# Guilucand/PanDelos

Measured on AMD Instinct MI355X. Metric: scored gene-pairs/sec (whole node), higher is better.
Workload: dtype u32 accumulate + f32 finalize

## Files before the change

pandelos_amd/csrc/pdl_api.hip:

```cpp
#include "pdl_common.h"

#include <algorithm>
#include <cstdlib>
#include <cstring>
#include <limits>

static thread_local std::string g_create_error = "";

enum class Lock { held, take };
template <class Body, class Undo>
static int guarded(pdl_ctx *c, Lock lock, Body &&body, Undo &&undo) {
    int code = PDL_ERR_DEVICE;
    std::string msg;
    try { return body(); }
    catch (const pdl_error &e) { code = e.code; msg = e.msg; }
    catch (const std::bad_alloc &) { msg = "host allocation failed"; }
    catch (const std::exception &e) { msg = e.what(); }
    undo();
    if (!c) g_create_error = msg;
    else if (lock == Lock::take) { std::lock_guard<std::mutex> lk(c->mu); c->err = msg; }
    else c->err = msg;
    return code;
}
template <class Body> static int guarded(pdl_ctx *c, Body &&body) { return guarded(c, Lock::held, body, [] {}); }
// ... 574 lines not shown
    memset(out, 0, sizeof(*out));
    std::lock_guard<std::mutex> lk(c->mu);
    return guarded(c, Lock::held, [&]() -> int {
        if ((n_edges && (!src || !dst)) || (n_sequences && !genome_of)) PDL_FAIL(PDL_ERR_ARGUMENT, "pdl_families_of_edges: NULL pointer");
        if (n_edges >= 0x7fffffffull || n_sequences >= 0x7fffffffu) PDL_FAIL(PDL_ERR_UNSUPPORTED, "pdl_families_of_edges: 2^31 genes or edges and more");
        PDL_HIP(hipSetDevice(c->device));
        pdl_ctx::FamBufs &b = c->fb;
        uint32_t g_max = 0;
        for (uint32_t i = 0; i < n_sequences; i++) g_max = std::max(g_max, genome_of[i]);
        if (n_edges) {
            b.up_src.alloc(n_edges * 4); b.up_dst.alloc(n_edges * 4);
            PDL_HIP(hipMemcpyAsync(b.up_src.p, src, n_edges * 4, hipMemcpyHostToDevice, c->stream));
            PDL_HIP(hipMemcpyAsync(b.up_dst.p, dst, n_edges * 4, hipMemcpyHostToDevice, c->stream));
        }
        if (n_sequences) {
            b.up_gen.alloc((size_t) n_sequences * 4);
            PDL_HIP(hipMemcpyAsync(b.up_gen.p, genome_of, (size_t) n_sequences * 4, hipMemcpyHostToDevice, c->stream));
        }
        const int32_t *s2[2] = {b.up_src.as<int32_t>(), nullptr}, *d2[2] = {b.up_dst.as<int32_t>(), nullptr};
        const uint64_t n2[2] = {n_edges, 0};
        pdl_fam_result r;
        pdl_run_families(c, s2, d2, n2, false, true, true, b.up_gen.as<uint32_t>(), n_sequences, bit_length64(g_max), r);
        fill_families(r, out);
        return PDL_OK;
    }, [&] { pdl_free_families(out); });
}

void pdl_free_placement(pdl_placement *p) {
    if (!p) return;
    free(p->src); free(p->dst); free(p->score); free(p->family_of); free(p->is_node); free(p->group_label); free(p->group_query_off);
    free(p->group_query); free(p->group_base_off); free(p->group_base); free(p->group_collides);
    memset(p, 0, sizeof(*p));
}

static void fill_placement(const pdl_place_result &r, bool with_edges, pdl_placement *out) {
    out->sequences = r.sequences; out->n_query = r.n_query; out->genomes = r.genomes;
    out->edges = (uint32_t) r.src.size(); out->edges_phase1 = r.edges_phase1; out->groups = r.groups;
    out->novel = r.novel; out->joined = r.joined; out->bridging = r.bridging; out->colliding = r.colliding; out->unplaced = r.unplaced;
    out->device_ms = r.device_ms;
    if (with_edges) { out->src = dup_vec(r.src); out->dst = dup_vec(r.dst); out->score = dup_vec(r.score); }
    out->family_of = dup_vec(r.family_of); out->is_node = dup_vec(r.is_node); out->group_label = dup_vec(r.group_label);
    out->group_query_off = dup_vec(r.group_query_off); out->group_query = dup_vec(r.group_query);
    out->group_base_off = dup_vec(r.group_base_off); out->group_base = dup_vec(r.group_base); out->group_collides = dup_vec(r.group_collides);
}

int pdl_place_query(pdl_ctx *c, const uint8_t *residues, const uint64_t *offsets, uint32_t n_query, pdl_placement *out, pdl_query_info *info) {
    if (!c) return PDL_ERR_ARGUMENT;
    std::lock_guard<std::mutex> lk(c->mu);
    if (out) memset(out, 0, sizeof(*out));
    if (info) memset(info, 0, sizeof(*info));
    return guarded(c, Lock::held, [&]() -> int {
        require_state(c, "pdl_place_query", NEEDS_WHOLE_SET, "pdl_placement_of_edges");
        if (!out) PDL_FAIL(PDL_ERR_ARGUMENT, "pdl_place_query: NULL pointer");
        check_genes("pdl_place_query", residues, offsets, n_query);
        int rc = c->scored ? PDL_OK : score_all_locked(c);
        if (rc != PDL_OK) return rc;
        PDL_HIP(hipSetDevice(c->device));
        if (!c->edges_valid) pdl_run_bbh_all(c);
        if (!c->fam_valid) pdl_run_families_of_context(c);
        pdl_place_result r;
        pdl_query_info qi{};
        pdl_run_place_query(c, residues, offsets, n_query, r, &qi);
        fill_placement(r, true, out);
        if (info) *info = qi;
        return PDL_OK;
    }, [&] { if (out) pdl_free_placement(out); if (info) memset(info, 0, sizeof(*info)); });
}

int pdl_placement_of_edges(pdl_ctx *c, const pdl_families *base, const uint32_t *genome_of, uint32_t n_query, const int32_t *src, const int32_t *dst,
                           uint64_t n_edges, pdl_placement *out) {
    if (!c || !out) return PDL_ERR_ARGUMENT;
    memset(out, 0, sizeof(*out));
    std::lock_guard<std::mutex> lk(c->mu);
    return guarded(c, Lock::held, [&]() -> int {
        if (!base || (n_edges && (!src || !dst))) PDL_FAIL(PDL_ERR_ARGUMENT, "pdl_placement_of_edges: NULL pointer");
        const uint32_t N = base->sequences, F = base->families, nodes = base->nodes;
        if (N && (!genome_of || !base->component_of || !base->is_node)) PDL_FAIL(PDL_ERR_ARGUMENT, "pdl_placement_of_edges: NULL pointer");
        if (!base->family_off || (nodes && !base->family_genes) || (F && !base->collides)) PDL_FAIL(PDL_ERR_ARGUMENT, "pdl_placement_of_edges: NULL pointer in the base families");
        if (n_query == 0) PDL_FAIL(PDL_ERR_ARGUMENT, "pdl_placement_of_edges: no query gene");
        if (n_edges >= 0x7fffffffull || (uint64_t) N + n_query >= 0x7fffffffull) PDL_FAIL(PDL_ERR_UNSUPPORTED, "pdl_placement_of_edges: 2^31 genes or edges and more");
        if (nodes > N || F > nodes || base->family_off[0] != 0 || base->family_off[F] != nodes) PDL_FAIL(PDL_ERR_ARGUMENT, "pdl_placement_of_edges: inconsistent base families (counts)");
        std::vector<uint32_t> of_label(N, 0);
        std::vector<uint8_t> listed(N, 0);
        for (uint32_t f = 0; f < F; f++) {
            const uint32_t a = base->family_off[f], b = base->family_off[f + 1];
            if (b <= a || b > nodes) PDL_FAIL(PDL_ERR_ARGUMENT, "pdl_placement_of_edges: inconsistent base families (family_off at %u)", f);
            const uint32_t label = base->family_genes[a];
            if (f && label <= base->family_genes[base->family_off[f - 1]])
                PDL_FAIL(PDL_ERR_ARGUMENT, "pdl_placement_of_edges: inconsistent base families (family %u is not behind family %u in label order)", f, f - 1);
            for (uint32_t j = a; j < b; j++) {
                const uint32_t g = base->family_genes[j];
                if (g >= N || listed[g] || !base->is_node[g] || base->component_of[g] != label || (j > a && g <= base->family_genes[j - 1]))
                    PDL_FAIL(PDL_ERR_ARGUMENT, "pdl_placement_of_edges: inconsistent base families (member %u of family %u)", j - a, f);
                listed[g] = 1;
            }
            of_label[label] = f;
        }
        uint32_t g_max = 0;
        for (uint32_t i = 0; i < N; i++) {
            g_max = std::max(g_max, genome_of[i]);
            if (base->is_node[i] ? !listed[i] : base->component_of[i] != i)
                PDL_FAIL(PDL_ERR_ARGUMENT, "pdl_placement_of_edges: inconsistent base families (gene %u)", i);
        }
        if (g_max >= 0x7fffffffu) PDL_FAIL(PDL_ERR_ARGUMENT, "pdl_placement_of_edges: genome id %u (ids below 2^31 - 1)", g_max);
        PDL_HIP(hipSetDevice(c->device));
        pdl_ctx::PlaceBufs &b = c->pb;
        hipStream_t st = c->stream;
        b.up_comp.alloc((size_t) N * 4); b.up_is_node.alloc(N); b.up_fam_of_label.alloc((size_t) N * 4); b.up_gen.alloc((size_t) N * 4);
        b.up_fam_off.alloc(((size_t) F + 1) * 4); b.up_fam_genes.alloc((size_t) nodes * 4); b.up_collides.alloc(F);
        if (N) {
            PDL_HIP(hipMemcpyAsync(b.up_comp.p, base->component_of, (size_t) N * 4, hipMemcpyHostToDevice, st));
            PDL_HIP(hipMemcpyAsync(b.up_is_node.p, base->is_node, N, hipMemcpyHostToDevice, st));
            PDL_HIP(hipMemcpyAsync(b.up_fam_of_label.p, of_label.data(), (size_t) N * 4, hipMemcpyHostToDevice, st));
            PDL_HIP(hipMemcpyAsync(b.up_gen.p, genome_of, (size_t) N * 4, hipMemcpyHostToDevice, st));
        }
        PDL_HIP(hipMemcpyAsync(b.up_fam_off.p, base->family_off, ((size_t) F + 1) * 4, hipMemcpyHostToDevice, st));
        if (nodes) PDL_HIP(hipMemcpyAsync(b.up_fam_genes.p, base->family_genes, (size_t) nodes * 4, hipMemcpyHostToDevice, st));
        if (F) PDL_HIP(hipMemcpyAsync(b.up_collides.p, base->collides, F, hipMemcpyHostToDevice, st));
        if (n_edges) {
            b.up_src.alloc(n_edges * 4); b.up_dst.alloc(n_edges * 4);
            PDL_HIP(hipMemcpyAsync(b.up_src.p, src, n_edges * 4, hipMemcpyHostToDevice, st));
            PDL_HIP(hipMemcpyAsync(b.up_dst.p, dst, n_edges * 4, hipMemcpyHostToDevice, st));
        }
        PlaceBase B;
        B.comp = b.up_comp.as<uint32_t>(); B.is_node = b.up_is_node.as<uint8_t>(); B.collides = b.up_collides.as<uint8_t>();
        B.fam_off = b.up_fam_off.as<uint32_t>(); B.fam_genes = b.up_fam_genes.as<uint32_t>(); B.fam_of_label = b.up_fam_of_label.as<uint32_t>();
        B.genome_of = b.up_gen.as<uint32_t>(); B.N = N; B.G = N ? g_max + 1 : 0;
        pdl_place_result r;
        pdl_run_place_edges(c, B, n_query, b.up_src.as<int32_t>(), b.up_dst.as<int32_t>(), n_edges, r);
        fill_placement(r, false, out);
        return PDL_OK;
    }, [&] { pdl_free_placement(out); });
}

int pdl_set_option(pdl_ctx *c, const char *name, int64_t value) {
    if (!c || !name) return PDL_ERR_ARGUMENT;
    std::lock_guard<std::mutex> lk(c->mu);
    const std::string n(name);
    if (n == "join_tier1") {
        if (!(value == -1 || value == 0 || (value >= 9 && value <= 11) || value == 20 || value == 21)) { c->err = "join_tier1: -1, 0, 9, 10, 11, 20 or 21"; return PDL_ERR_ARGUMENT; }
        c->opt_tier1 = (int) value;
    } else if (n == "join_tier0") c->opt_tier0 = value < 0 ? -1 : (value != 0);
    else if (n == "sift_threshold") {
        if (value != 0 && value != 1) { c->err = "sift_threshold: 0 or 1"; return PDL_ERR_ARGUMENT; }
        c->opt_sift_threshold = (int) value;
    }
    else if (n == "join_tiny_tier2") c->opt_tiny_tier2 = value != 0;
    else if (n == "join_grid_pct") c->opt_grid_pct = (int) value;
    else if (n == "stage_timers") c->opt_stage_timers = value != 0;
    else if (n == "host_mirror") c->opt_host_mirror = value != 0;
    else if (n == "staging_cap") c->opt_staging_cap = value > 0 ? (uint64_t) value : 0;
    else if (n == "aside_test_reload") c->opt_aside_test_reload = value != 0;
    else if (n == "onepass_scan") c->opt_onepass_scan = value != 0;
    else if (n == "low_memory") c->opt_low_memory = value != 0;
    else if (n == "query_batch_bytes") {
        if (value <= 0) { c->err = "query_batch_bytes: a positive byte count"; return PDL_ERR_ARGUMENT; }
        c->opt_query_batch_bytes = (uint64_t) value;
        return PDL_OK;
    }
    else { c->err = "unknown option " + n; return PDL_ERR_ARGUMENT; }
    c->scored = false;
    return PDL_OK;
}

int pdl_dist_preprocess_begin(pdl_ctx *c, const uint8_t *d_residues, const uint64_t *d_offsets, const uint32_t *d_genome_of,
                              uint32_t n, uint64_t n_res, int k, uint32_t world, uint32_t rank, pdl_dist_slice *out) {
    if (!c || !out) return PDL_ERR_ARGUMENT;
    std::lock_guard<std::mutex> lk(c->mu);
    return guarded(c, [&]() -> int {
    if (!d_offsets || !d_genome_of || (!d_residues && n_res)) PDL_FAIL(PDL_ERR_ARGUMENT, "null input pointer");
    if (((uintptr_t) d_residues & 15) != 0) PDL_FAIL(PDL_ERR_ARGUMENT, "d_residues must be 16-byte aligned");
    if (world == 0 || rank >= world || world > 64) PDL_FAIL(PDL_ERR_ARGUMENT, "rank %u of %u (at most 64 ranks)", rank, world);
    PDL_HIP(hipSetDevice(c->device));
    c->preprocessed = false; c->scored = false; c->tasks_ready = false; c->mirror_valid = false;
    c->dist = false; c->dist_stage = 0;
    adopt_device_input(c, d_residues, d_offsets, d_genome_of, n, n_res);
    c->N = n; c->R = n_res;
    c->U = c->Ushared = c->NG = c->P = c->M = 0;
    if (k <= 0) PDL_FAIL(PDL_ERR_KVALUE, "K value must be greater than 0.");
    if (n == 0) PDL_FAIL(PDL_ERR_EMPTY, "empty dataset");
    build_genome_layout(c);
    c->world = world; c->rank = rank;
    c->shard.clear(); c->shard_set = false; c->dict_shard.clear();
    pdl_run_dist_begin(c, k);
    out->d_postings = c->post.p; out->records = c->U_slice; out->kmers = c->M_slice;
    out->genome_weights = c->h_run_weights.data(); out->genomes = c->G;
    out->genome_costs = c->h_run_costs.data();
    return PDL_OK;
    });
}

int pdl_dist_preprocess_finish(pdl_ctx *c, void *d_postings_all, uint64_t total_records, const uint64_t *genome_weights, pdl_cost *out_cost) {
    if (!c) return PDL_ERR_ARGUMENT;
    std::lock_guard<std::mutex> lk(c->mu);
    return guarded(c, [&]() -> int {
    if (!c->dist || c->dist_stage != 1) PDL_FAIL(PDL_ERR_STATE, "pdl_dist_preprocess_finish without pdl_dist_preprocess_begin");
    if (c->dist_sender) PDL_FAIL(PDL_ERR_STATE, "pdl_dist_preprocess_ranges built this run's range tuples (and took its group-head bits out): finish with pdl_dist_preprocess_finish_ranges");
    if (!d_postings_all || ((uintptr_t) d_postings_all & 7) != 0) PDL_FAIL(PDL_ERR_ARGUMENT, "the gathered dictionary must be an 8-byte aligned device array");
    if (total_records < c->U_slice) PDL_FAIL(PDL_ERR_ARGUMENT, "the gathered dictionary (%llu records) is smaller than this rank's run (%llu)",
                                             (unsigned long long) total_records, (unsigned long long) c->U_slice);
    PDL_HIP(hipSetDevice(c->device));
    c->post_ext = static_cast<uint2 *>(d_postings_all);
    pdl_run_dist_finish(c, total_records, genome_weights);
    c->preprocessed = true;
    fill_cost(c, out_cost);
    return PDL_OK;
    });
}

int pdl_dist_preprocess_ranges(pdl_ctx *c, const uint64_t *run_records, const uint64_t *genome_weights, const uint64_t *genome_costs, pdl_dist_ranges *out) {
    if (!c || !out || !run_records || !genome_weights || !genome_costs) return PDL_ERR_ARGUMENT;
    std::lock_guard<std::mutex> lk(c->mu);
    return guarded(c, [&]() -> int {
    if (!c->dist || c->dist_stage != 1) PDL_FAIL(PDL_ERR_STATE, "pdl_dist_preprocess_ranges without pdl_dist_preprocess_begin");
    PDL_HIP(hipSetDevice(c->device));
    memset(out, 0, sizeof(*out));
    out->available = pdl_run_dist_ranges(c, run_records, genome_weights, genome_costs) ? 1 : 0;
    out->d_keys = c->dist_out_keys; out->d_ranges = reinterpret_cast<const uint64_t *>(c->dist_out_ranges);
    out->counts = c->h_tuple_counts.data(); out->total = c->dist_out_total;
    out->shared_records = c->dist_run_counters[0]; out->groups = c->dist_run_counters[1]; out->repeat_sample = c->dist_run_counters[2];
    return PDL_OK;
    });
}

int pdl_dist_preprocess_finish_ranges(pdl_ctx *c, void *d_postings_all, uint64_t total_records, uint32_t *d_keys, uint64_t *d_ranges, uint64_t n_tuples,
                                      const uint64_t *counter_sums, pdl_cost *out_cost) {
    if (!c || !counter_sums || ((!d_keys || !d_ranges) && n_tuples)) return PDL_ERR_ARGUMENT;
    std::lock_guard<std::mutex> lk(c->mu);
    return guarded(c, [&]() -> int {
    if (!c->dist || c->dist_stage != 1 || !c->dist_sender) PDL_FAIL(PDL_ERR_STATE, "pdl_dist_preprocess_finish_ranges without a pdl_dist_preprocess_ranges that said \"available\"");
    if (!d_postings_all || ((uintptr_t) d_postings_all & 7) != 0) PDL_FAIL(PDL_ERR_ARGUMENT, "the gathered dictionary must be an 8-byte aligned device array");
    if (n_tuples && ((((uintptr_t) d_keys) & 3) != 0 || (((uintptr_t) d_ranges) & 7) != 0)) PDL_FAIL(PDL_ERR_ARGUMENT, "the received tuples must be aligned device arrays");
    PDL_HIP(hipSetDevice(c->device));
    c->post_ext = static_cast<uint2 *>(d_postings_all);
    pdl_run_dist_finish_ranges(c, total_records, d_keys, reinterpret_cast<unsigned long long *>(d_ranges), n_tuples, counter_sums);
    c->preprocessed = true;
    fill_cost(c, out_cost);
    return PDL_OK;
    });
}

int pdl_dist_genome_owner(const pdl_ctx *c, uint32_t *out) {
    if (!c || !out) return PDL_ERR_ARGUMENT;
    if (!c->dist || c->dist_stage < 2) return PDL_ERR_STATE;
    memcpy(out, c->h_owner.data(), (size_t) c->G * 4);
    return PDL_OK;
}

int pdl_dist_score_begin(pdl_ctx *c, pdl_dist_outbox *out) {
    if (!c || !out) return PDL_ERR_ARGUMENT;
    std::lock_guard<std::mutex> lk(c->mu);
    return guarded(c, [&]() -> int {
    if (!c->dist || c->dist_stage < 2) PDL_FAIL(PDL_ERR_STATE, "pdl_dist_score_begin before pdl_dist_preprocess_finish");
    PDL_HIP(hipSetDevice(c->device));
    c->scored = false; c->mirror_valid = false; c->edges_valid = false; c->dist_stage = 2;
    pdl_run_dist_score_begin(c);
    out->d_cells = c->outbox.as<pdl_dist_cell>();
    out->counts = c->h_outbox_counts.data();
    out->total = 0;
    for (uint64_t v : c->h_outbox_counts) out->total += v;
    return PDL_OK;
    });
}

int pdl_dist_score_finish(pdl_ctx *c, const pdl_dist_cell *d_inbox, uint64_t n_inbox) {
    if (!c || (!d_inbox && n_inbox)) return PDL_ERR_ARGUMENT;
    std::lock_guard<std::mutex> lk(c->mu);
    return guarded(c, [&]() -> int {
    if (!c->dist || c->dist_stage != 3) PDL_FAIL(PDL_ERR_STATE, "pdl_dist_score_finish without pdl_dist_score_begin");
    if (n_inbox >= 0xffffffffull) PDL_FAIL(PDL_ERR_UNSUPPORTED, "more than 2^32 received cells");
    PDL_HIP(hipSetDevice(c->device));
    pdl_run_dist_score_finish(c, d_inbox, n_inbox);
    return PDL_OK;
    });
}

int pdl_copy_device(pdl_ctx *c, void *d_dst, const void *d_src, uint64_t bytes) {
    if (!c || ((!d_dst || !d_src) && bytes)) return PDL_ERR_ARGUMENT;
    std::lock_guard<std::mutex> lk(c->mu);
    return guarded(c, [&]() -> int {
    PDL_HIP(hipSetDevice(c->device));
    if (bytes) PDL_HIP(hipMemcpyAsync(d_dst, d_src, bytes, hipMemcpyDeviceToDevice, c->stream));
    PDL_HIP(hipStreamSynchronize(c->stream));
    return PDL_OK;
    });
}

int pdl_get_dictionary(pdl_ctx *c, uint64_t *ranks, uint32_t *seqs, uint32_t *counts) {
    if (!c) return PDL_ERR_ARGUMENT;
    std::lock_guard<std::mutex> lk(c->mu);
    return guarded(c, [&]() -> int {
    if (!c->preprocessed) PDL_FAIL(PDL_ERR_STATE, "pdl_get_dictionary before pdl_preprocess");
    if (c->dist) PDL_FAIL(PDL_ERR_STATE, "pdl_get_dictionary: a multi-GPU context keeps ranks only for its own interval");
    if (!c->keys_b.p || !c->recpos.p) PDL_FAIL(PDL_ERR_STATE, "pdl_get_dictionary: the sorted k-mer stream was released (option low_memory)");
    PDL_HIP(hipSetDevice(c->device));
    const uint64_t U = c->U, M = c->M;
    std::vector<uint32_t> recpos(U);
    std::vector<uint2> post(U);
    PDL_HIP(hipMemcpyAsync(recpos.data(), c->recpos.p, U * 4, hipMemcpyDeviceToHost, c->stream));
    PDL_HIP(hipMemcpyAsync(post.data(), c->post.p, U * 8, hipMemcpyDeviceToHost, c->stream));
    std::vector<uint8_t> keys(M * (c->key64 ? 8 : 4));
    PDL_HIP(hipMemcpyAsync(keys.data(), c->keys_b.p, keys.size(), hipMemcpyDeviceToHost, c->stream));
    PDL_HIP(hipStreamSynchronize(c->stream));
    for (uint64_t u = 0; u < U; u++) {
        if (ranks) ranks[u] = c->key64 ? reinterpret_cast<uint64_t *>(keys.data())[recpos[u]]
                                       : (uint64_t) reinterpret_cast<uint32_t *>(keys.data())[recpos[u]];
// ... 123 lines not shown
```

pandelos_amd/csrc/pdl_common.h:

```cpp
#pragma once

#include <atomic>
#include <chrono>

#include <hip/hip_runtime.h>

#include <algorithm>
#include <cstdint>
#include <cstdio>
#include <mutex>
#include <cstdlib>
#include <new>
#include <string>
#include <utility>
#include <vector>

#include "../../include/pandelos_amd.h"

#define PDL_WAVE 64

#ifdef __HIPCC__
__device__ __forceinline__ void pdl_sync() {
#ifndef PDL_PLAIN_SYNCTHREADS
    asm volatile("s_waitcnt lgkmcnt(0)" ::: "memory");
// ... 111 lines not shown
    size_t bytes = 0;
    void alloc(size_t n) {
        if (n <= bytes && p) return;
        release();
        size_t want = n ? n : 16;
        PDL_HIP(hipMalloc(&p, want));
        bytes = want;
    }
    void release() {
        if (p) (void) hipFree(p);
        p = nullptr;
        bytes = 0;
    }
    template <class T> T *as() const { return static_cast<T *>(p); }
    ~DevBuf() { release(); }
    void grow_keep(size_t n, hipStream_t st) {
        if (n <= bytes && p) return;
        void *q = nullptr;
        PDL_HIP(hipMalloc(&q, n));
        if (p && bytes) {
            PDL_HIP(hipMemcpyAsync(q, p, bytes, hipMemcpyDeviceToDevice, st));
            PDL_HIP(hipStreamSynchronize(st));
            (void) hipFree(p);
        }
        p = q;
        bytes = n;
    }
    void swap(DevBuf &o) { std::swap(p, o.p); std::swap(bytes, o.bytes); }
    DevBuf() = default;
    DevBuf(const DevBuf &) = delete;
    DevBuf &operator=(const DevBuf &) = delete;
};

struct DevView {
    void *p = nullptr;
    template <class T> T *as() const { return static_cast<T *>(p); }
};

struct RankParams {
    uint8_t rank_values[256];
    uint64_t last_multiplier;
    uint32_t base;
    uint32_t k;
    uint32_t rank_bits;
    uint32_t hash_fallback;
    uint32_t key_bits;
};

struct EventPair {
    hipEvent_t a = nullptr, b = nullptr;
    bool used = false;
};

template <int N> struct EventSpans {
    hipEvent_t ev[2 * N] = {};
    hipStream_t st = nullptr;
    int n = 0;
    void start(hipStream_t s) { st = s; n = 0; for (hipEvent_t &e : ev) if (!e) PDL_HIP(hipEventCreate(&e)); }
    void begin() { PDL_HIP(hipEventRecord(ev[2 * n], st)); }
    void end() { PDL_HIP(hipEventRecord(ev[2 * n + 1], st)); n++; }
    float ms(int i) const { float v = 0.f; return i < n && hipEventElapsedTime(&v, ev[2 * i], ev[2 * i + 1]) == hipSuccess ? v : 0.f; }
    float total_ms() const { float total = 0.f; for (int i = 0; i < n; i++) total += ms(i); return total; }
    EventSpans() = default;
    EventSpans(const EventSpans &) = delete;
    EventSpans &operator=(const EventSpans &) = delete;
    ~EventSpans() { for (hipEvent_t e : ev) if (e) (void) hipEventDestroy(e); }
};
using QSpans = EventSpans<3>;
template <class T> inline void pdl_renew(T &x) { x.~T(); new (&x) T(); }

struct pdl_fam_result {
    uint32_t sequences = 0, nodes = 0, families = 0, colliding = 0;
    std::vector<uint32_t> component_of, family_off, family_genes;
    std::vector<uint8_t> is_node, collides;
    float device_ms = 0.f;
};

struct pdl_place_result {
    uint32_t sequences = 0, n_query = 0, genomes = 0, edges_phase1 = 0, groups = 0;
    uint32_t novel = 0, joined = 0, bridging = 0, colliding = 0, unplaced = 0;
    std::vector<int32_t> src, dst;
    std::vector<float> score;
    std::vector<uint32_t> family_of, group_label, group_query_off, group_query, group_base_off, group_base;
    std::vector<uint8_t> is_node, group_collides;
    float device_ms = 0.f;
};
struct PlaceBase {
    const uint32_t *comp = nullptr, *fam_off = nullptr, *fam_genes = nullptr, *fam_of_label = nullptr, *genome_of = nullptr;
    const uint8_t *is_node = nullptr, *collides = nullptr;
    uint32_t N = 0, G = 0;
};
struct pdl_query_run {
    uint64_t Z = 0, cap = 1, residues = 0, kmers = 0, records = 0, matched = 0, cost = 0;
};

struct pdl_ctx {
    int device = 0;
    hipStream_t stream = nullptr;
    bool own_stream = false;
    uint32_t flags = 0;
    std::string err;
    std::mutex mu;

    const uint8_t *d_res = nullptr;
    const uint64_t *d_off = nullptr;
    const uint32_t *d_gen = nullptr;
    DevBuf in_res, in_off, in_gen;
    DevBuf own_gen;

    uint32_t *gen_pin = nullptr; size_t gen_pin_words = 0;
    hipEvent_t ev_gen = nullptr;
    bool layout_deferred = false;

    bool preprocessed = false;
    bool only_complexity = false;
    uint32_t N = 0, G = 0;
    uint64_t R = 0, M = 0, U = 0, Ushared = 0, NG = 0, P = 0, sum_kseq = 0, max_kseq = 0, min_kseq = 0;
    uint64_t Urepeat = 0;
    RankParams rp{};

    DevBuf ing_res, ing_off, ing_gen;
    uint8_t *ing_pin[2] = {nullptr, nullptr};
    size_t ing_pin_bytes = 0;
    hipEvent_t ing_ev[2] = {nullptr, nullptr};
    hipStream_t ing_stream = nullptr;
    std::vector<uint64_t> ing_h_off;
    std::vector<uint32_t> ing_h_gen;
    std::vector<std::string> ing_genome_names;
    uint64_t ing_R = 0;
    bool ingested = false;

    DevBuf kseq_len;
    DevBuf gene_len;
    DevBuf kmer_off;
    DevBuf cost;
    std::vector<uint64_t> h_genome_cost;

    DevBuf keys_a, keys_b, vals_a, vals_b, sort_tmp;
    bool key64 = false;
    DevBuf recpos;
    DevBuf post;
    DevBuf ranges;
    const uint2 *ranges8 = nullptr;
    DevBuf head_bits;
    bool costs_ready = true;
    DevBuf seq_off;
    bool upper_only = false;
    DevBuf scan_tmp;
    DevBuf lb_tile, lb_chunk, lb_ctr;
    uint32_t lb_epoch = 0;
    bool opt_low_memory = false;
    bool reshard_pending = false;
    bool opt_onepass_scan = false;
    DevBuf scratch;
    DevBuf scalars;

    std::vector<uint32_t> h_genome_of;
    std::vector<uint32_t> h_genome_row_off;
    std::vector<uint32_t> h_genome_rows;
    std::vector<uint32_t> shard;
    bool shard_set = false;
    std::vector<uint32_t> dict_shard;
    DevBuf seq_in_shard;
    DevBuf own_iv;
    std::vector<uint2> h_own_iv;
    std::vector<uint8_t> h_seq_in_shard;

    bool scored = false;
    uint32_t n_task_rows = 0;
    std::vector<int32_t> h_local_genome;
    std::vector<uint32_t> h_task_row_off;
    std::vector<uint64_t> h_cell_off;
    DevBuf task_blob;
    uint32_t *task_pin = nullptr; size_t task_pin_words = 0;
    hipStream_t copy_stream = nullptr; hipEvent_t ev_tasks = nullptr, ev_entry = nullptr;
    DevView task_rows;
    DevView task_lg;
    DevBuf row_desc;
    DevBuf MS;
    DevBuf CM;
    DevBuf row_base, row_cnt, fin_off;
    DevBuf st_score, st_perc, st_tr, st_col, st_first;
    uint64_t st_cap = 0;
    DevBuf c_score, c_perc, c_tr, c_row, c_col;
    uint64_t Z = 0;
    DevBuf join_ctr;
    DevBuf overflow_rows;
    DevBuf gene_info;
    DevBuf join_defer;
    DevBuf glb_table;
    bool glb_clean = false;
    DevBuf row_desc2;
    DevBuf mirror_cnt, mirror_ref;
    DevView taskpos_of;
    std::vector<uint32_t> h_fin;
    bool tasks_ready = false;
    DevBuf scratch2;
    DevBuf task_off;
    int cus = 0;
    uint32_t occ_tier1[5] = {0, 0, 0, 0, 0};
    uint32_t occ_tier0[2] = {0, 0}, occ_tier0b[2] = {0, 0};

    bool edges_valid = false;
    DevBuf bbh_kind, bbh_tab, e_src, e_dst, e_score;
    uint8_t *edge_mirror = nullptr;
    size_t edge_mirror_bytes = 0;
    uint64_t n_edges = 0, n_edges1 = 0;
    std::vector<uint32_t> h_bbh_at;
    std::vector<uint64_t> h_edge1, h_edge_off;

    int opt_tier1 = -1;
    int opt_tier0 = -1;
    int opt_sift_threshold = 1;
    bool opt_tiny_tier2 = false;
    bool opt_stage_timers = true;
    int opt_grid_pct = 0;
    bool opt_host_mirror = true;
    uint64_t opt_staging_cap = 0;
    bool opt_aside_test_reload = false;

    bool dist = false;
    uint32_t world = 1, rank = 0;
    int dist_stage = 0;
    uint2 *post_ext = nullptr;
    uint64_t U_slice = 0, M_slice = 0;
    std::vector<uint32_t> h_owner;
    std::vector<uint64_t> h_upper_cost;
    std::vector<uint64_t> h_run_weights;
    std::vector<uint64_t> h_run_costs;
    bool dist_sender = false;
    int dist_tail = -1;
    uint64_t run_base = 0, dist_total = 0;
    DevBuf seq_owner;
    DevBuf tuple_off;
    std::vector<uint64_t> h_tuple_counts;
    uint32_t *dist_out_keys = nullptr;
    unsigned long long *dist_out_ranges = nullptr;
    uint64_t dist_out_total = 0, dist_run_counters[3] = {0, 0, 0};
    DevBuf owner_of_genome;
    DevView local_genome;
    DevBuf outbox;
    DevBuf outbox_tab;
    std::vector<uint64_t> h_outbox_counts;
    uint64_t st_local = 0;
    uint64_t n_inbox = 0;
    uint32_t order_grid1 = 0;

    struct QueryBufs {
        DevBuf res, off, koff, kseq, keys_a, keys_b, vals_a, vals_b, recpos, post, desc, gkey, rec_sorted, row_lookups, row_off,
               fold, ctl, MS, CM, row_base, row_cnt, fin_off, rowid, overflow, st, cells, hbm;
        bool hbm_clean = false;
        uint32_t hbm_cols = 0, hbm_slots = 0;
        const uint32_t *rec_sorted_at = nullptr;
        QSpans spans;
    } qb;
    struct QueryBatchBufs {
        DevBuf res, off, koff, kseq, gene_begin, res_begin, gene_query, keys_a, keys_b, vals_a, vals_b, recpos, post, qkey, perm, srank, spost,
               seg_off, folds, desc, gkey, rec_sorted, row_lookups, row_off, ctl, MS, CM, row_base, row_cnt, fin_off, rowid, overflow, st, cells;
        QSpans spans;
        uint8_t *stage = nullptr; size_t stage_bytes = 0;
        ~QueryBatchBufs() { if (stage) (void) hipHostFree(stage); }
    } qbb;
    uint64_t opt_query_batch_bytes = 1ull << 30;
    struct FamBufs {
        DevBuf parent, comp, same_deg, is_node, collides, fam_off, fam_of_label, run_off, run_of;
        DevBuf mk_a, mk_b, mv_a, mv_b;
        DevBuf ck_a, ck_b, cv_a, cv_b;
        DevBuf ek_a, ek_b, ev_a, ev_b;
        DevBuf up_src, up_dst, up_gen;
        EventSpans<2> spans;
    } fb;
    bool fam_valid = false;
    pdl_fam_result fam;
    uint64_t fam_serial = 0;
    struct PlaceBufs {
        DevBuf base_comp, base_is_node, base_collides, base_fam_off, base_fam_genes, base_fam_of_label;
        uint64_t base_serial = 0;
        DevBuf up_comp, up_is_node, up_collides, up_fam_off, up_fam_genes, up_fam_of_label, up_gen, up_src, up_dst;
        DevBuf ctl;
        DevBuf kind, tab, e_src, e_dst, e_score;
        DevBuf parent, is_node, same_deg, family_of, gcol, grp_of_label, gq_off, gb_off, group_base, mpre;
        DevBuf mk_a, mk_b, mv_a, mv_b;
        DevBuf bk_a, bk_b, bv_a, bv_b, uniq;
        DevBuf ek_a, ek_b, ev_a, ev_b;
        QSpans spans;
    } pb;
    EventSpans<2> app_spans;
    struct RemoveBufs {
        DevBuf gmap;
        DevBuf gen_in;
        DevBuf new_id;
        DevBuf kseq, gen, glen;
        DevBuf tile;
        DevBuf ctl;
        EventSpans<2> spans;
    } rm;
    uint8_t alpha_present[256] = {};

    pdl_timings tm{};
    EventPair ev[16];
    uint8_t *pin = nullptr;
    uint8_t *pin_dev = nullptr;
    size_t pin_bytes = 0;
    uint32_t pin_epoch = 0;
    uint8_t *mirror = nullptr;
    size_t mirror_bytes = 0;
// ... 199 lines not shown
```

pandelos_amd/csrc/pdl_dict.hip:

```cpp
#include "pdl_common.h"
#include "pdl_scan.h"
#include "pdl_sort.h"
#include "pdl_append.h"
#include "pdl_remove.h"
#include "pdl_groups.h"

#include <algorithm>
#include <cstring>

#define RABIN_MODULO 18446744073709551557ULL


__global__ __launch_bounds__(256) void k_zero_u64(uint64_t *p, size_t n) {
    for (size_t i = (size_t) blockIdx.x * 256 + threadIdx.x; i < n; i += (size_t) gridDim.x * 256) p[i] = 0;
}
constexpr int HIST_THREADS = 256;
__global__ __launch_bounds__(HIST_THREADS) void k_hist(const uint8_t *__restrict__ res, uint64_t n, unsigned long long *__restrict__ hist) {
    __shared__ uint32_t s_seen[256];
    s_seen[threadIdx.x] = 0;
    pdl_sync();
    const uint64_t n16 = n / 16;
    const uint4 *res16 = reinterpret_cast<const uint4 *>(res);
    const uint64_t stride = (uint64_t) gridDim.x * HIST_THREADS;
    auto mark = [&](const uint4 &v) {
        const uint32_t w[4] = {v.x, v.y, v.z, v.w};
#pragma unroll
        for (int j = 0; j < 4; j++) {
            s_seen[w[j] & 0xff] = 1u; s_seen[(w[j] >> 8) & 0xff] = 1u; s_seen[(w[j] >> 16) & 0xff] = 1u; s_seen[w[j] >> 24] = 1u;
        }
    };
    uint64_t i = (uint64_t) blockIdx.x * HIST_THREADS + threadIdx.x;
    for (; i + 3 * stride < n16; i += 4 * stride) {
        const uint4 v0 = res16[i], v1 = res16[i + stride], v2 = res16[i + 2 * stride], v3 = res16[i + 3 * stride];
        mark(v0); mark(v1); mark(v2); mark(v3);
    }
    for (; i < n16; i += stride) mark(res16[i]);
    if (blockIdx.x == 0)
        for (uint64_t t = n16 * 16 + threadIdx.x; t < n; t += HIST_THREADS) s_seen[res[t]] = 1u;
    pdl_sync();
    if (s_seen[threadIdx.x]) hist[threadIdx.x] = 1ull;
}

static void rank_init_host(RankParams &rp, const uint64_t counters[256], int kvalue) {
    memset(&rp, 0, sizeof(rp));
    rp.k = (uint32_t) kvalue;
    int rank = 0;
    for (int i = 0; i < 256; i++)
        if (counters[i] > 0) rp.rank_values[i] = (uint8_t) rank++;
    const uint8_t rank_base = (uint8_t) rank;
    rp.base = rank_base;
    uint64_t last_multiplier = 1;
    bool has_overflow = false;
    int tmp_kvalue = kvalue - 1;
    while (tmp_kvalue--) {
        uint64_t ovflw_test = last_multiplier;
        last_multiplier *= rank_base;
        if (has_overflow) {
            last_multiplier %= RABIN_MODULO;
        } else if ((ovflw_test > last_multiplier) || (ovflw_test * rank_base > last_multiplier * rank_base)) {
            has_overflow = true;
            last_multiplier = ((ovflw_test % RABIN_MODULO) * rank_base) % RABIN_MODULO;
        }
    }
    rp.last_multiplier = last_multiplier;
    rp.hash_fallback = has_overflow ? 1u : 0u;
    rp.key_bits = 64;
    if (has_overflow) {
        rp.rank_bits = 64;
    } else {
        uint64_t rank_tmp = last_multiplier * rank_base;
        rp.rank_bits = rank_tmp ? bit_length64(rank_tmp - 1) : 1;
        if (rp.rank_bits == 0) rp.rank_bits = 1;
        unsigned __int128 exact = 1;
        bool fits = true;
        for (int i = 0; i < kvalue && fits; i++) { exact *= rank_base; fits = (exact >> 64) == 0; }
        if (fits) rp.key_bits = rp.rank_bits;
    }
}

struct KseqFlag {
    const uint64_t *off; uint32_t k;
    __device__ uint32_t operator()(uint64_t i) const {
        const uint64_t b = off[i], e = off[i + 1];
        const uint64_t len = e >= b ? e - b : 0;
        return len >= k ? (uint32_t) (len - k + 1) : 0u;
    }
};
struct KseqApply {
    uint32_t *kseq_len; uint32_t *gene_len; uint64_t *kmer_off;
    unsigned long long *cost;
    const uint64_t *off; uint64_t n_res; unsigned long long *bad;
    __device__ void operator()(uint64_t i, uint32_t f, uint32_t prefix) const {
        kseq_len[i] = f;
        gene_len[i] = (uint32_t) (off[i + 1] - off[i]);
        kmer_off[i] = prefix;
        cost[i] = 0;
        if (off[i + 1] < off[i] || off[i + 1] > n_res) atomicOr(bad, 1ull);
    }
};

constexpr uint32_t RANK_SPAN = 128;
constexpr int RANK_THREADS = 256;
constexpr int RANK_ITEMS = 4;
constexpr int RANK_TILE = RANK_THREADS * RANK_ITEMS;

__device__ __forceinline__ uint32_t upper_bound_u64(const uint64_t *a, uint32_t lo, uint32_t hi, uint64_t v) {
    while (lo < hi) {
        uint32_t mid = lo + ((hi - lo) >> 1);
        if (a[mid] <= v) lo = mid + 1; else hi = mid;
    }
    return lo;
}

struct __attribute__((packed, aligned(1))) UnalignedU64 { uint64_t v; };
__device__ __forceinline__ uint64_t load_residues8(const uint8_t *__restrict__ res, uint64_t p, uint64_t n_res) {
    if (p + 8 <= n_res) return reinterpret_cast<const UnalignedU64 *>(res + p)->v;
    uint64_t w = 0;
    for (uint32_t b = 0; b < 8 && p + b < n_res; b++) w |= (uint64_t) res[p + b] << (8 * b);
    return w;
}

constexpr uint32_t DIST_BIN_BITS = 12, DIST_BINS = 1u << DIST_BIN_BITS;

template <class KeyT, int MODE>
__global__ __launch_bounds__(RANK_THREADS) void k_rank(const uint8_t *__restrict__ res, const uint64_t *__restrict__ off,
                                                       const uint64_t *__restrict__ kmer_off, uint32_t n_seq, uint64_t m, uint64_t n_res,
                                                       RankParams rp, KeyT *__restrict__ keys, uint32_t *__restrict__ vals,
                                                       uint32_t bin_shift, uint32_t *__restrict__ bins) {
    __shared__ uint8_t s_rv[256];
    __shared__ uint32_t s_lo, s_hi;
    __shared__ uint64_t s_koff[RANK_SPAN + 1], s_off[RANK_SPAN];
    __shared__ uint32_t s_bins[MODE == 1 ? DIST_BINS : 1];
    for (int i = threadIdx.x; i < 256; i += RANK_THREADS) s_rv[i] = rp.rank_values[i];
    if constexpr (MODE == 1) for (uint32_t i = threadIdx.x; i < DIST_BINS; i += RANK_THREADS) s_bins[i] = 0;
    const uint64_t tiles = (m + RANK_TILE - 1) / RANK_TILE;
  for (uint64_t tile = blockIdx.x; tile < tiles; tile += gridDim.x) {
    pdl_sync();
    const uint64_t q0 = tile * RANK_TILE;
    const uint64_t q_last = min(q0 + RANK_TILE, m) - 1;
    if (threadIdx.x == 0) s_lo = upper_bound_u64(kmer_off, 0, n_seq + 1, q0) - 1;
    if (threadIdx.x == 64) s_hi = upper_bound_u64(kmer_off, 0, n_seq + 1, q_last) - 1;
    pdl_sync();
    const uint32_t lo = s_lo, hi = s_hi;
    const uint32_t span = hi - lo + 1;
    const bool staged = span <= RANK_SPAN;
    if (staged) {
        for (uint32_t i = threadIdx.x; i <= span; i += RANK_THREADS) s_koff[i] = kmer_off[lo + i];
        for (uint32_t i = threadIdx.x; i < span; i += RANK_THREADS) s_off[i] = off[lo + i];
    }
    pdl_sync();
    const uint32_t k = rp.k;
    const KeyT base = (KeyT) rp.base;
    uint32_t sq[RANK_ITEMS];
    uint64_t pos[RANK_ITEMS];
#pragma unroll
    for (int j = 0; j < RANK_ITEMS; j++) {
        const uint64_t qj = q0 + (uint64_t) j * RANK_THREADS + threadIdx.x;
        const uint64_t q = qj < m ? qj : m - 1;
        if (staged) {
            uint32_t a = 0;
            if (span <= 8) {
#pragma unroll
                for (uint32_t i = 1; i < 8; i++) a += (uint32_t) (i < span && s_koff[i < span ? i : 0] <= q);
            } else {
                uint32_t b = span;
                while (a < b) { const uint32_t mid = (a + b) >> 1; if (s_koff[mid + 1] <= q) a = mid + 1; else b = mid; }
            }
            sq[j] = lo + a;
            pos[j] = s_off[a] + (q - s_koff[a]);
        } else {
            sq[j] = upper_bound_u64(kmer_off, lo, hi + 1, q) - 1;
            pos[j] = off[sq[j]] + (q - kmer_off[sq[j]]);
        }
    }
    KeyT r[RANK_ITEMS];
#pragma unroll
    for (int j = 0; j < RANK_ITEMS; j++) r[j] = 0;
    for (uint32_t c0 = 0; c0 < k; c0 += 8) {
        uint64_t w[RANK_ITEMS];
        bool safe = true;
#pragma unroll
        for (int j = 0; j < RANK_ITEMS; j++) safe = safe && pos[j] + c0 + 8 <= n_res;
        if (__all(safe)) {
#pragma unroll
            for (int j = 0; j < RANK_ITEMS; j++) w[j] = reinterpret_cast<const UnalignedU64 *>(res + pos[j] + c0)->v;
        } else {
#pragma unroll
            for (int j = 0; j < RANK_ITEMS; j++) w[j] = load_residues8(res, pos[j] + c0, n_res);
        }
        const uint32_t nb = min(8u, k - c0);
        for (uint32_t b = 0; b < nb; b++) {
#pragma unroll
            for (int j = 0; j < RANK_ITEMS; j++) r[j] = r[j] * base + s_rv[(uint32_t) (w[j] >> (8 * b)) & 0xffu];
        }
    }
#pragma unroll
    for (int j = 0; j < RANK_ITEMS; j++) {
        const uint64_t q = q0 + (uint64_t) j * RANK_THREADS + threadIdx.x;
        if (q < m) {
            if constexpr (MODE == 1) atomicAdd(&s_bins[(uint32_t) (r[j] >> bin_shift)], 1u);
            keys[q] = r[j]; vals[q] = sq[j];
        }
    }
  }
    if constexpr (MODE == 1) {
        pdl_sync();
        for (uint32_t i = threadIdx.x; i < DIST_BINS; i += RANK_THREADS) { const uint32_t v = s_bins[i]; if (v) atomicAdd(&bins[i], v); }
    }
}

__device__ __forceinline__ uint64_t update_rank_hash_dev(uint64_t current, uint64_t vnext, uint64_t vpop, uint64_t lm, uint64_t base) {
    uint64_t wrapped = current + RABIN_MODULO - vpop * lm;
    uint64_t lo = wrapped * base;
    uint64_t hi = __umul64hi(wrapped, base);
    uint64_t lo2 = lo + vnext;
    hi += (lo2 < lo);
    uint64_t t = hi * 59ull;
    uint64_t r = lo2 + t;
    if (r < lo2) r += 59ull;
    if (r >= RABIN_MODULO) r -= RABIN_MODULO;
    return r;
}

template <int MODE>
__global__ __launch_bounds__(256) void k_rank_hash(const uint8_t *__restrict__ res, const uint64_t *__restrict__ off,
                                                   const uint64_t *__restrict__ kmer_off, uint32_t n_seq, RankParams rp,
                                                   uint64_t *__restrict__ keys, uint32_t *__restrict__ vals, uint32_t *__restrict__ bins) {
    __shared__ uint8_t s_rv[256];
    for (int i = threadIdx.x; i < 256; i += 256) s_rv[i] = rp.rank_values[i];
    pdl_sync();
    const uint32_t s = blockIdx.x * 256 + threadIdx.x;
    if (s >= n_seq) return;
    const uint64_t b = off[s], e = off[s + 1];
    const uint32_t k = rp.k;
    if (e - b < k) return;
    const uint8_t *p = res + b;
    const uint64_t len = e - b;
    uint64_t q = kmer_off[s];
    uint64_t rank = 0;
    const uint64_t v0 = s_rv[0];
    for (uint32_t i = 0; i < k; i++) rank = update_rank_hash_dev(rank, s_rv[p[i]], v0, rp.last_multiplier, rp.base);
    if constexpr (MODE == 1) atomicAdd(&bins[rank >> (64 - DIST_BIN_BITS)], 1u);
    keys[q] = rank; vals[q] = s; q++;
    for (uint64_t i = k; i < len; i++) {
        rank = update_rank_hash_dev(rank, s_rv[p[i]], s_rv[p[i - k]], rp.last_multiplier, rp.base);
        if constexpr (MODE == 1) atomicAdd(&bins[rank >> (64 - DIST_BIN_BITS)], 1u);
        keys[q] = rank; vals[q] = s; q++;
    }
}

template <class KeyT> struct RecHead {
    const KeyT *keys; const uint32_t *vals;
    __device__ uint32_t operator()(uint64_t q) const {
        const uint64_t qp = q ? q - 1 : 0;
        const KeyT k0 = keys[q], k1 = keys[qp];
        const uint32_t v0 = vals[q], v1 = vals[qp];
        return (uint32_t) (q == 0) | (uint32_t) (k0 != k1) | (uint32_t) (v0 != v1);
    }
};
template <class KeyT> struct RecScatter {
    const KeyT *keys; const uint32_t *vals; uint64_t m;
    uint32_t *recpos; uint2 *post;
    struct Loaded { uint32_t val, run; uint8_t head; };
    __device__ Loaded load(uint64_t q, uint32_t) const {
        const uint64_t qp = q ? q - 1 : 0, qn = q + 1 < m ? q + 1 : q;
        const KeyT key = keys[q], kprev = keys[qp], knext = keys[qn];
        const uint32_t val = vals[q], vnext = vals[qn];
        const bool head = q == 0 || kprev != key;
        uint64_t j = q + 1;
        if (j < m && knext == key && vnext == val) {
            j++;
            while (j < m && keys[j] == key && vals[j] == val) j++;
        }
        return Loaded{val, (uint32_t) (j - q), (uint8_t) (head ? 1 : 0)};
    }
    __device__ void store(uint64_t q, uint32_t f, uint32_t prefix, const Loaded &v) const {
        if (!f) return;
        recpos[prefix] = (uint32_t) q;
        post[prefix] = make_uint2(v.val, v.run | ((uint32_t) v.head << 31));
    }
};

template <class KeyT> struct SelFlag {
    const KeyT *keys; uint32_t shift, b_lo, b_hi;
    __device__ uint32_t operator()(uint64_t q) const { const uint32_t b = (uint32_t) (keys[q] >> shift); return (uint32_t) (b >= b_lo) & (uint32_t) (b < b_hi); }
};
template <class KeyT> struct SelApply {
    const KeyT *keys; const uint32_t *vals; KeyT *keys_out; uint32_t *vals_out;
    struct Loaded { KeyT key; uint32_t val; };
    __device__ Loaded load(uint64_t q, uint32_t f) const { return f ? Loaded{keys[q], vals[q]} : Loaded{0, 0u}; }
    __device__ void store(uint64_t, uint32_t f, uint32_t prefix, const Loaded &v) const { if (f) { keys_out[prefix] = v.key; vals_out[prefix] = v.val; } }
};

__global__ __launch_bounds__(256) void k_genes_of_rank(const uint32_t *__restrict__ genome_of, const uint32_t *__restrict__ owner, uint32_t rank,
                                                       uint32_t n_seq, uint8_t *__restrict__ in_shard) {
    const uint32_t s = blockIdx.x * 256 + threadIdx.x;
    if (s < n_seq) in_shard[s] = owner[genome_of[s]] == rank ? 1 : 0;
}
__global__ __launch_bounds__(256) void k_gene_owner(const uint32_t *__restrict__ genome_of, const uint32_t *__restrict__ owner, uint32_t n_seq,
                                                    uint8_t *__restrict__ seq_owner) {
    const uint32_t s = blockIdx.x * 256 + threadIdx.x;
    if (s < n_seq) seq_owner[s] = (uint8_t) owner[genome_of[s]];
}
__global__ __launch_bounds__(256) void k_owner_keys(uint32_t *__restrict__ key, const uint64_t *d_n, const uint8_t *__restrict__ seq_owner) {
    const uint32_t n = (uint32_t) *d_n;
    for (uint32_t i = blockIdx.x * 256 + threadIdx.x; i < n; i += gridDim.x * 256) {
        const uint32_t g = key[i];
        key[i] = g | ((uint32_t) seq_owner[g] << 24);
    }
}

__global__ __launch_bounds__(256) void k_gather_ranges(const uint32_t *__restrict__ idx_sorted, const uint32_t *__restrict__ key_sorted,
                                                       const uint4 *__restrict__ tuples, const uint64_t *d_n, uint4 *__restrict__ ranges,
                                                       unsigned long long *__restrict__ cost) {
    const uint32_t n = (uint32_t) *d_n;
    const uint32_t e = blockIdx.x * 256 + threadIdx.x;
    if (blockIdx.x * 256u >= n) return;
    const uint32_t lane = threadIdx.x & (PDL_WAVE - 1);
    const bool live = e < n;
    uint32_t g = 0xffffffffu;
    unsigned long long w = 0;
    if (live) {
        const uint4 t = tuples[idx_sorted[e]];
        ranges[e] = t;
        g = key_sorted[e];
        w = t.w;
    }
    unsigned long long todo = __ballot(live);
    while (todo) {
        const int leader = __ffsll((long long) todo) - 1;
        const uint32_t gl = __shfl(g, leader, PDL_WAVE);
        const bool in = live && g == gl;
        unsigned long long sum = in ? w : 0ull;
#pragma unroll
        for (int d = PDL_WAVE / 2; d > 0; d >>= 1) sum += __shfl_xor(sum, d, PDL_WAVE);
        if ((int) lane == leader) atomicAdd(&cost[gl], sum);
        todo &= ~__ballot(in);
    }
}
__global__ __launch_bounds__(256) void k_seq_offsets(const uint32_t *__restrict__ key_sorted, const uint64_t *d_n, uint32_t n_seq,
                                                     uint32_t *__restrict__ seq_off, uint32_t shift = 0, uint32_t mask = 0xffffffffu) {
    const uint32_t n = (uint32_t) *d_n;
    const uint32_t s = blockIdx.x * 256 + threadIdx.x;
    if (s > n_seq) return;
    uint32_t lo = 0, hi = n;
    while (lo < hi) {
        uint32_t mid = lo + ((hi - lo) >> 1);
        if (((key_sorted[mid] >> shift) & mask) < s) lo = mid + 1; else hi = mid;
    }
    seq_off[s] = lo;
}

__global__ __launch_bounds__(256) void k_genome_cost(const unsigned long long *__restrict__ cost, const uint32_t *__restrict__ kseq_len,
                                                     const uint32_t *__restrict__ genome_of, uint32_t n_seq,
                                                     unsigned long long *__restrict__ genome_cost, unsigned long long *__restrict__ sum_kseq,
                                                     unsigned long long *__restrict__ max_kseq, unsigned long long *__restrict__ min_kseq) {
    __shared__ unsigned long long s_sum, s_max, s_min;
    if (threadIdx.x == 0) { s_sum = 0; s_max = 0; s_min = ~0ull; }
    pdl_sync();
    const uint32_t lane = threadIdx.x & (PDL_WAVE - 1);
    unsigned long long ksum = 0, kmax = 0, kmin = ~0ull;
    for (uint32_t s0 = blockIdx.x * 256; s0 < n_seq; s0 += gridDim.x * 256) {
        const uint32_t s = s0 + threadIdx.x;
        const bool live = s < n_seq;
        unsigned long long c = live ? cost[s] : 0ull;
        const unsigned long long kl = live ? (unsigned long long) kseq_len[s] : 0ull;
        const uint32_t g = live ? genome_of[s] : 0xffffffffu;
        ksum += kl; kmax = kl > kmax ? kl : kmax; if (kl && kl < kmin) kmin = kl;
        const uint32_t g0 = __shfl(g, 0, PDL_WAVE);
        if (__all(g == g0 || !live)) {
            unsigned long long csum = c;
#pragma unroll
            for (int d = PDL_WAVE / 2; d > 0; d >>= 1) csum += __shfl_down(csum, d, PDL_WAVE);
            if (lane == 0 && csum && g0 != 0xffffffffu) atomicAdd(&genome_cost[g0], csum);
        } else if (live && c) {
            atomicAdd(&genome_cost[g], c);
        }
    }
#pragma unroll
    for (int d = PDL_WAVE / 2; d > 0; d >>= 1) {
        ksum += __shfl_down(ksum, d, PDL_WAVE);
        unsigned long long o = __shfl_down(kmax, d, PDL_WAVE);
        kmax = o > kmax ? o : kmax;
        o = __shfl_down(kmin, d, PDL_WAVE);
        kmin = o < kmin ? o : kmin;
    }
    if (lane == 0) { atomicAdd(&s_sum, ksum); atomicMax(&s_max, kmax); atomicMin(&s_min, kmin); }
    pdl_sync();
    if (threadIdx.x == 0 && s_sum) { atomicAdd(sum_kseq, s_sum); atomicMax(max_kseq, s_max); atomicMax(min_kseq, ~s_min); }
}

static void launch_genome_cost(pdl_ctx *c, size_t w_sum, size_t w_max) {
    static_assert(PDL_CTL_KSEQ_NMIN == PDL_CTL_KSEQ_MAX + 1 && PDL_CTL_LAZY_KSEQ_MAX + 1 <= PDL_CTL_LAST, "~min sits behind max");
    unsigned long long *d_scal = c->scalars.as<unsigned long long>();
    hipLaunchKernelGGL(k_genome_cost, dim3(std::min<uint32_t>((c->N + 255) / 256, 128)), dim3(256), 0, c->stream, c->cost.as<unsigned long long>(),
                       c->kseq_len.as<uint32_t>(), c->d_gen, c->N, d_scal + PDL_CTL_GCOST, d_scal + w_sum, d_scal + w_max, d_scal + w_max + 1);
    PDL_HIP(hipGetLastError());
}


static void stage_alphabet_and_lengths(pdl_ctx *c, int kvalue, bool only_complexity) {
    hipStream_t st = c->stream;
    if (kvalue <= 0) PDL_FAIL(PDL_ERR_KVALUE, "K value must be greater than 0.");
    const size_t ctl_words = PDL_CTL_GCOST + 2 * (size_t) (c->layout_deferred ? c->N : c->G);
    c->scalars.alloc(ctl_words * sizeof(uint64_t));
    uint64_t *d_scal = c->scalars.as<uint64_t>();
    hipLaunchKernelGGL(k_zero_u64, dim3((uint32_t) std::min<size_t>((ctl_words + 255) / 256, 1024)), dim3(256), 0, st, d_scal, ctl_words);

    ev_begin(c, EV_HIST);
    c->kseq_len.alloc((size_t) c->N * sizeof(uint32_t));
    c->gene_len.alloc((size_t) c->N * sizeof(uint32_t));
    c->kmer_off.alloc(((size_t) c->N + 1) * sizeof(uint64_t));
    c->cost.alloc((size_t) c->N * sizeof(uint64_t));
    scan_and_apply(c, c->N, KseqFlag{c->d_off, (uint32_t) kvalue},
                   KseqApply{c->kseq_len.as<uint32_t>(), c->gene_len.as<uint32_t>(), c->kmer_off.as<uint64_t>(), c->cost.as<unsigned long long>(), c->d_off, c->R,
                             reinterpret_cast<unsigned long long *>(d_scal + PDL_CTL_BAD_OFFSETS)}, d_scal + PDL_CTL_KMERS, c->kmer_off.as<uint64_t>() + c->N);
    if (c->layout_deferred) pdl_input_arrived(c);
    if (c->R) {
        uint32_t blocks = (uint32_t) std::min<uint64_t>((c->R / 64 + HIST_THREADS - 1) / HIST_THREADS + 1, 2048);
        hipLaunchKernelGGL(k_hist, dim3(blocks), dim3(HIST_THREADS), 0, st, c->d_res, c->R,
                           reinterpret_cast<unsigned long long *>(d_scal + PDL_CTL_HIST));
    }
    uint64_t counters[256];
    uint64_t M = 0, bad = 0;
    {
        PinRead rd(c);
        const uint64_t *pc = rd.add<uint64_t>(d_scal, PDL_CTL_GCOST);
        ev_end(c, EV_HIST);
        rd.sync();
        memcpy(counters, pc + PDL_CTL_HIST, sizeof(counters));
        M = pc[PDL_CTL_KMERS]; bad = pc[PDL_CTL_BAD_OFFSETS];
    }
    if (bad) PDL_FAIL(PDL_ERR_ARGUMENT, "offsets must ascend from 0 to the residue count (%llu)", (unsigned long long) c->R);
    rank_init_host(c->rp, counters, kvalue);
    for (int i = 0; i < 256; i++) c->alpha_present[i] = counters[i] ? 1 : 0;
    c->M = M;
    c->only_complexity = only_complexity;
    if (M == 0) PDL_FAIL(PDL_ERR_EMPTY, "no gene is at least k=%d residues long: the dictionary is empty", kvalue);
    if (c->R >= 0xfffffff0ull) PDL_FAIL(PDL_ERR_UNSUPPORTED, "more than 2^32 residues (%llu) need 64-bit stream positions", (unsigned long long) c->R);
    c->key64 = c->rp.rank_bits > 32;
}

template <class KeyT>
static void stage_rank(pdl_ctx *c, uint32_t *d_bins = nullptr, uint32_t bin_shift = 0) {
    hipStream_t st = c->stream;
    const uint64_t M = c->M;
    c->keys_a.alloc(M * sizeof(KeyT)); c->keys_b.alloc(M * sizeof(KeyT));
    c->vals_a.alloc(M * sizeof(uint32_t)); c->vals_b.alloc(M * sizeof(uint32_t));
    if (c->rp.hash_fallback) {
        if constexpr (sizeof(KeyT) == 8) {
            if (d_bins) hipLaunchKernelGGL(k_rank_hash<1>, dim3((c->N + 255) / 256), dim3(256), 0, st, c->d_res, c->d_off,
                                           c->kmer_off.as<uint64_t>(), c->N, c->rp, c->keys_a.as<uint64_t>(), c->vals_a.as<uint32_t>(), d_bins);
            else hipLaunchKernelGGL(k_rank_hash<0>, dim3((c->N + 255) / 256), dim3(256), 0, st, c->d_res, c->d_off,
                                    c->kmer_off.as<uint64_t>(), c->N, c->rp, c->keys_a.as<uint64_t>(), c->vals_a.as<uint32_t>(), (uint32_t *) nullptr);
        }
    } else {
        const uint64_t tiles = (M + RANK_TILE - 1) / RANK_TILE;
        if (d_bins) hipLaunchKernelGGL((k_rank<KeyT, 1>), dim3((uint32_t) std::min<uint64_t>(tiles, 2048)), dim3(RANK_THREADS), 0, st, c->d_res, c->d_off,
                                       c->kmer_off.as<uint64_t>(), c->N, M, c->R, c->rp, c->keys_a.as<KeyT>(), c->vals_a.as<uint32_t>(), bin_shift, d_bins);
        else hipLaunchKernelGGL((k_rank<KeyT, 0>), dim3((uint32_t) tiles), dim3(RANK_THREADS), 0, st, c->d_res, c->d_off,
                                c->kmer_off.as<uint64_t>(), c->N, M, c->R, c->rp, c->keys_a.as<KeyT>(), c->vals_a.as<uint32_t>(), 0u, (uint32_t *) nullptr);
    }
    PDL_HIP(hipGetLastError());
}

template <class KeyT>
static void stage_dedup(pdl_ctx *c, uint64_t m) {
    uint64_t *d_scal = c->scalars.as<uint64_t>();
    const KeyT *skeys = c->keys_b.as<KeyT>();
    const uint32_t *svals = c->vals_b.as<uint32_t>();
    ev_begin(c, EV_DICT);
    c->recpos.alloc((m + 1) * sizeof(uint32_t));
    c->post.alloc(m * sizeof(uint2));
    scan_and_apply(c, m, RecHead<KeyT>{skeys, svals},
                   RecScatter<KeyT>{skeys, svals, m, c->recpos.as<uint32_t>(), c->post.as<uint2>()}, d_scal + PDL_CTL_RECORDS);
}

template <class KeyT>
static void stage_sort_and_dedup(pdl_ctx *c, KeyT *keys_in, KeyT *keys_out, uint32_t *vals_in, uint32_t *vals_out, uint64_t m) {
    ev_begin(c, EV_SORT1);
    pdl_sort_pairs<KeyT>(c, keys_in, keys_out, vals_in, vals_out, m, c->rp.rank_bits, false, nullptr, 0, c->rp.key_bits == c->rp.rank_bits);
    ev_end(c, EV_SORT1);
    if ((void *) keys_out != c->keys_b.p) c->keys_a.swap(c->keys_b);
    if ((void *) vals_out != c->vals_b.p) c->vals_a.swap(c->vals_b);
    stage_dedup<KeyT>(c, m);
}

static void group_shard_args(pdl_ctx *c, GroupTileArgs &ga) {
    hipStream_t st = c->stream;
    std::vector<uint2> &iv = c->h_own_iv;
    iv.clear();
    bool contiguous = true;
    for (uint32_t g : c->dict_shard) {
        const uint32_t b0 = c->h_genome_row_off[g], e0 = c->h_genome_row_off[g + 1];
        if (b0 == e0) continue;
        const uint32_t first = c->h_genome_rows[b0], last = c->h_genome_rows[e0 - 1];
        if (last - first + 1 != e0 - b0) { contiguous = false; break; }
        if (!iv.empty() && iv.back().y == first) iv.back().y = last + 1; else iv.push_back(make_uint2(first, last + 1));
    }
    if (contiguous) std::sort(iv.begin(), iv.end(), [](const uint2 &p, const uint2 &q) { return p.x < q.x; });
    for (size_t i = 1; contiguous && i < iv.size(); i++) if (iv[i].x < iv[i - 1].y) contiguous = false;
    if (contiguous && !iv.empty() && iv.size() <= GW_MAX_IV) {
        c->own_iv.alloc(iv.size() * sizeof(uint2));
        PDL_HIP(hipMemcpyAsync(c->own_iv.p, iv.data(), iv.size() * sizeof(uint2), hipMemcpyHostToDevice, st));
        ga.own_iv = c->own_iv.as<uint2>(); ga.n_own_iv = (uint32_t) iv.size();
    }
    if (!c->dist) {
        std::vector<uint8_t> &h = c->h_seq_in_shard;
        h.assign((size_t) c->N, 0);
        std::vector<uint8_t> gsel((size_t) c->G, 0);
        for (uint32_t g : c->dict_shard) gsel[g] = 1;
        for (uint32_t i = 0; i < c->N; i++) h[i] = gsel[c->h_genome_of[i]];
        c->seq_in_shard.alloc(c->N);
        PDL_HIP(hipMemcpyAsync(c->seq_in_shard.p, h.data(), c->N, hipMemcpyHostToDevice, st));
    }
    ga.in_shard = c->seq_in_shard.as<uint8_t>();
}

static void stage_ranges_and_costs(pdl_ctx *c, uint64_t bound, int mode, bool only_complexity) {
    hipStream_t st = c->stream;
    c->costs_ready = true; c->ranges8 = nullptr;
    uint64_t *d_scal = c->scalars.as<uint64_t>();
    const uint64_t *d_u = d_scal + PDL_CTL_RECORDS;
    uint2 *post = pdl_postings(c);
    GroupTileArgs ga{};
    ga.post = post; ga.n_bound = bound; ga.d_n = d_u;
    const uint32_t grid = group_tiles_plan(c, ga);
    ga.cost = c->cost.as<unsigned long long>();
    ga.counters = reinterpret_cast<unsigned long long *>(d_scal + PDL_CTL_COUNTERS);
    ga.genome_of = c->d_gen; ga.n_genomes = c->G;
    hipLaunchKernelGGL(k_fold_last_record, dim3(1), dim3(1024), 0, st, post, c->post_ext ? (uint32_t *) nullptr : c->recpos.as<uint32_t>(), d_u);
    if (only_complexity) {
        launch_group_costs<false, true>(c, ga, grid);
    } else {
        ev_begin(c, EV_SORT2);
        const bool packed = mode != 0 && c->N < (1u << 22);
        const bool exact = mode != 1;
        uint64_t cap = bound;
        uint4 *tuples = nullptr;
        unsigned long long *pay_a = nullptr, *pay_b = nullptr;
        uint32_t *k2a = nullptr, *v2a = nullptr, *k2b = nullptr, *v2b = nullptr;
        auto carve = [&]() {
            c->scratch.alloc(cap * (packed ? 2 * sizeof(uint64_t) + sizeof(uint32_t) : sizeof(uint4) + 3 * sizeof(uint32_t)) + (exact ? cap * sizeof(uint32_t) : 0) + 64);
            tuples = c->scratch.as<uint4>();
            pay_a = c->scratch.as<unsigned long long>(); pay_b = pay_a + cap;
            v2a = packed ? nullptr : reinterpret_cast<uint32_t *>(tuples + cap);
            k2b = packed ? reinterpret_cast<uint32_t *>(pay_b + cap) : v2a + cap;
            v2b = packed ? nullptr : k2b + cap;
            if (exact) k2a = (packed ? k2b : v2b) + cap;
            else { c->vals_a.alloc(cap * sizeof(uint32_t)); k2a = c->vals_a.as<uint32_t>(); }
        };
        if (!exact) carve();
        if (mode != 1) group_shard_args(c, ga);
        c->head_bits.alloc(((bound + GW_TILE - 1) / GW_TILE) * GW_ROUNDS * sizeof(uint64_t));
        ga.head_bits = c->head_bits.as<unsigned long long>();
        const uint64_t *d_us = d_scal + PDL_CTL_RANGES;
        const bool fused = mode == 1 && packed;
        if (fused) {
            const uint32_t n_tiles4 = (uint32_t) ((bound + PDL_RADIX_TILE - 1) / PDL_RADIX_TILE);
            const size_t table = (size_t) PDL_RADIX_BINS * n_tiles4, tiles = (bound + GW_TILE - 1) / GW_TILE;
            c->sort_tmp.alloc((2 * table + 3 * tiles + 1) * sizeof(uint32_t));
            uint32_t *counts = c->sort_tmp.as<uint32_t>(), *offs = counts + table;
            ga.tile_sums = offs + table; ga.th_first = ga.tile_sums + tiles; ga.th_last = ga.th_first + tiles; ga.chunk_sums = nullptr;
            const uint32_t grid4 = std::max<uint32_t>(1, std::min<uint32_t>(n_tiles4, (uint32_t) c->cus * 8));
            hipLaunchKernelGGL(k_range_count_hist, dim3(grid4), dim3(GW_THREADS), 0, st, ga, n_tiles4, counts);
            pdl_radix_offsets(c, counts, offs, n_tiles4, d_scal + PDL_CTL_RANGES);
            hipLaunchKernelGGL(k_range_scatter, dim3(n_tiles4), dim3(GW_THREADS), 0, st, ga, n_tiles4, offs, k2b, pay_b);
            PDL_HIP(hipGetLastError());
        } else {
        launch_range_count(c, ga, grid, mode);
        if (exact) {
            if (!c->tasks_ready) pdl_prepare_tasks(c);
            PinRead rd(c);
            const uint64_t *pn = rd.add<uint64_t>(d_us, 1);
            rd.sync();
            cap = std::max<uint64_t>(pn[0], 1);
            carve();
        }
        ga.key2 = k2a; ga.tuples = tuples; ga.pay8 = packed ? pay_a : nullptr;
        launch_range_write(c, ga, grid, mode);
        }
        c->upper_only = mode != 0;
        const uint32_t seq_bits = std::max<uint32_t>(1, bit_length64(c->N ? c->N - 1 : 0));
        uint64_t n_sort = bound;
        const uint64_t *d_sort_n = d_us;
        if (exact) { n_sort = cap; d_sort_n = nullptr; }
        c->seq_off.alloc(((size_t) c->N + 1) * sizeof(uint32_t));
        if (packed) {
            if (fused) {
                std::swap(k2a, k2b); std::swap(pay_a, pay_b);
                pdl_sort_pairs<uint32_t, unsigned long long>(c, k2a, k2b, pay_a, pay_b, n_sort, seq_bits, false, d_sort_n, 8, true);
            } else
            pdl_sort_pairs<uint32_t, unsigned long long>(c, k2a, k2b, pay_a, pay_b, n_sort, seq_bits, false, d_sort_n, 0, true);
            ev_end(c, EV_SORT2);
            ev_begin(c, EV_RANGES);
            c->ranges8 = reinterpret_cast<const uint2 *>(pay_b);
            c->costs_ready = false;
        } else {
            pdl_sort_pairs<uint32_t>(c, k2a, k2b, v2a, v2b, n_sort, seq_bits, true, d_sort_n, 0, true);
            ev_end(c, EV_SORT2);
            ev_begin(c, EV_RANGES);
            c->ranges8 = nullptr;
            c->ranges.alloc(std::max<uint64_t>(n_sort, 1) * sizeof(uint4));
            const uint32_t gblocks = (uint32_t) std::max<uint64_t>((n_sort + 255) / 256, 1);
            hipLaunchKernelGGL(k_gather_ranges, dim3(gblocks), dim3(256), 0, st, v2b, k2b, tuples, d_us, c->ranges.as<uint4>(), c->cost.as<unsigned long long>());
        }
        hipLaunchKernelGGL(k_seq_offsets, dim3((c->N + 1 + 255) / 256), dim3(256), 0, st, k2b, d_us, c->N, c->seq_off.as<uint32_t>());
        PDL_HIP(hipGetLastError());
        ev_end(c, EV_RANGES);
    }

    launch_genome_cost(c, PDL_CTL_KSEQ_SUM, PDL_CTL_KSEQ_MAX);

    uint64_t own_cost = 0;
    {
        PinRead rd(c);
        const uint64_t *pt = rd.add<uint64_t>(d_scal, PDL_CTL_GCOST + (size_t) c->G);
        const uint32_t *lbe = lookback_error_word(c, rd);
        rd.sync();
        lookback_check(c, lbe);
        c->h_genome_cost.assign(pt + PDL_CTL_GCOST, pt + PDL_CTL_GCOST + c->G);
        c->U = pt[PDL_CTL_RECORDS];
        c->Ushared = pt[PDL_CTL_SHARED];
        c->Urepeat = pt[PDL_CTL_REPEATS];
        c->NG = pt[PDL_CTL_GROUPS];
        c->sum_kseq = pt[PDL_CTL_KSEQ_SUM];
        c->max_kseq = pt[PDL_CTL_KSEQ_MAX];
        c->min_kseq = pt[PDL_CTL_KSEQ_NMIN] == 0 ? 1 : ~pt[PDL_CTL_KSEQ_NMIN];
        own_cost = pt[PDL_CTL_OWN_COST];
    }
    c->P = 0;
    if (c->costs_ready) for (uint64_t v : c->h_genome_cost) c->P += v;
    else c->P = own_cost;
}

void pdl_run_reshard(pdl_ctx *c) {
    hipStream_t st = c->stream;
    if (c->dist || c->post_ext) PDL_FAIL(PDL_ERR_STATE, "genome shard: a multi-GPU context deals the genomes itself");
    if (c->dict_shard.empty() || c->upper_only) PDL_FAIL(PDL_ERR_STATE, "genome shard: the dictionary was built for all genomes; set the first shard before pdl_preprocess");
    uint64_t *d_scal = c->scalars.as<uint64_t>();
    const uint32_t n = (uint32_t) c->U;
    ev_begin(c, EV_PRE_TOTAL);
    hipLaunchKernelGGL(k_restore_heads, dim3((n + 255) / 256), dim3(256), 0, st, c->post.as<uint2>(), c->head_bits.as<unsigned long long>(), n);
    PDL_HIP(hipMemsetAsync(d_scal + PDL_CTL_RANGES, 0, sizeof(uint64_t), st));
    PDL_HIP(hipMemsetAsync(d_scal + PDL_CTL_COUNTERS, 0, (PDL_CTL_LAST - PDL_CTL_COUNTERS + 1) * sizeof(uint64_t), st));
    PDL_HIP(hipMemsetAsync(d_scal + PDL_CTL_GCOST, 0, 2 * (size_t) c->G * sizeof(uint64_t), st));
    PDL_HIP(hipMemsetAsync(c->cost.p, 0, (size_t) c->N * sizeof(uint64_t), st));
    const uint64_t sum_kseq = c->sum_kseq, max_kseq = c->max_kseq, min_kseq = c->min_kseq;
    PDL_HIP(hipMemsetAsync(d_scal + PDL_CTL_KSEQ_SUM, 0, sizeof(uint64_t), st));
    PDL_HIP(hipMemsetAsync(d_scal + PDL_CTL_KSEQ_MAX, 0, (PDL_CTL_KSEQ_NMIN - PDL_CTL_KSEQ_MAX + 1) * sizeof(uint64_t), st));
    c->dict_shard = c->shard;
    c->tasks_ready = false;
    ev_begin(c, EV_DICT); ev_end(c, EV_DICT);
    stage_ranges_and_costs(c, c->U, 0, false);
    c->sum_kseq = sum_kseq; c->max_kseq = max_kseq; c->min_kseq = min_kseq;
    ev_end(c, EV_PRE_TOTAL);
    PDL_HIP(hipStreamSynchronize(st));
    c->tm.sort_seq_ms = ev_ms(c, EV_SORT2);
    c->tm.ranges_ms = ev_ms(c, EV_RANGES);
    c->tm.reshard_ms = ev_ms(c, EV_PRE_TOTAL);
}

void pdl_ensure_costs(pdl_ctx *c) {
    if (c->costs_ready) return;
    hipStream_t st = c->stream;
    uint64_t *d_scal = c->scalars.as<uint64_t>();
    PDL_HIP(hipMemsetAsync(c->cost.p, 0, (size_t) c->N * sizeof(uint64_t), st));
    PDL_HIP(hipMemsetAsync(d_scal + PDL_CTL_GCOST, 0, (size_t) c->G * sizeof(uint64_t), st));
    const uint32_t n = (uint32_t) c->U;
    hipLaunchKernelGGL(k_gene_costs_lazy, dim3((n + 255) / 256), dim3(256), 0, st, pdl_postings(c), c->head_bits.as<unsigned long long>(), n,
                       c->cost.as<unsigned long long>());
    launch_genome_cost(c, PDL_CTL_LAZY_KSEQ_SUM, PDL_CTL_LAZY_KSEQ_MAX);
    PinRead rd(c);
    const uint64_t *pg = rd.add<uint64_t>(d_scal + PDL_CTL_GCOST, c->G);
    rd.sync();
    c->h_genome_cost.assign(pg, pg + c->G);
    c->costs_ready = true;
}

static void release_build_buffers(pdl_ctx *c) {
    c->keys_a.release(); c->keys_b.release(); c->vals_a.release(); c->vals_b.release(); c->recpos.release(); c->sort_tmp.release();
}

template <class KeyT>
static void dictionary_pipeline(pdl_ctx *c, bool only_complexity) {
    const uint64_t M = c->M;
    ev_begin(c, EV_RANK);
    stage_rank<KeyT>(c);
    ev_end(c, EV_RANK);
    KeyT *keys_in = c->keys_a.as<KeyT>(), *keys_out = c->keys_b.as<KeyT>();
    uint32_t *vals_in = c->vals_a.as<uint32_t>(), *vals_out = c->vals_b.as<uint32_t>();
    stage_sort_and_dedup<KeyT>(c, keys_in, keys_out, vals_in, vals_out, M);
    ev_end(c, EV_DICT);
    if (c->layout_deferred) pdl_finish_layout(c);
    if (!only_complexity) pdl_prepare_tasks(c);
    stage_ranges_and_costs(c, M, c->dict_shard.empty() ? 1 : 0, only_complexity);
    if (c->opt_low_memory) {
        PDL_HIP(hipStreamSynchronize(c->stream));
        release_build_buffers(c);
    }
}

static void context_changes(pdl_ctx *c) {
    c->preprocessed = false; c->scored = false; c->tasks_ready = false; c->reshard_pending = false;
    c->mirror_valid = false; c->edges_valid = false; c->fam_valid = false;
}

template <class QueueStream>
static void rebuild_behind_sort(pdl_ctx *c, EventSpans<2> &spans, uint64_t M1, uint32_t N1, uint32_t G1, QueueStream &&queue_stream) {
    hipStream_t st = c->stream;
    const size_t ctl_words = PDL_CTL_GCOST + 2 * (size_t) G1;
    c->scalars.alloc(ctl_words * sizeof(uint64_t));
    c->cost.alloc((size_t) N1 * sizeof(uint64_t));
    spans.begin();
    hipLaunchKernelGGL(k_zero_u64, dim3((uint32_t) std::min<size_t>((ctl_words + 255) / 256, 1024)), dim3(256), 0, st, c->scalars.as<uint64_t>(), ctl_words);
    hipLaunchKernelGGL(k_zero_u64, dim3((uint32_t) std::min<size_t>(((size_t) N1 + 255) / 256, 1024)), dim3(256), 0, st, c->cost.as<uint64_t>(), (size_t) N1);
    PDL_HIP(hipGetLastError());
    queue_stream();
    if (c->key64) stage_dedup<uint64_t>(c, M1); else stage_dedup<uint32_t>(c, M1);
    ev_end(c, EV_DICT);
    pdl_prepare_tasks(c);
    stage_ranges_and_costs(c, M1, 1, false);
    spans.end();
    PDL_HIP(hipStreamSynchronize(st));
    if (c->opt_low_memory) release_build_buffers(c);
}

template <class KeyT>
static void rank_new_genes(pdl_ctx *c, const uint8_t *res, const uint64_t *off, const uint64_t *kmer_off, uint32_t n, uint64_t m, uint64_t n_res,
                           KeyT *keys, uint32_t *vals) {
    hipStream_t st = c->stream;
    if (c->rp.hash_fallback) {
        if constexpr (sizeof(KeyT) == 8)
            hipLaunchKernelGGL(k_rank_hash<0>, dim3((n + 255) / 256), dim3(256), 0, st, res, off, kmer_off, n, c->rp, keys, vals, (uint32_t *) nullptr);
    } else {
        const uint64_t tiles = (m + RANK_TILE - 1) / RANK_TILE;
        hipLaunchKernelGGL((k_rank<KeyT, 0>), dim3((uint32_t) tiles), dim3(RANK_THREADS), 0, st, res, off, kmer_off, n, m, n_res, c->rp,
                           keys, vals, 0u, (uint32_t *) nullptr);
    }
    PDL_HIP(hipGetLastError());
}

template <class KeyT>
static const void *query_dictionary(pdl_ctx *c, const uint8_t *res, const uint64_t *off, const uint64_t *kmer_off, uint32_t n, uint64_t m,
                                    uint64_t n_res, KeyT *keys_in, KeyT *keys_out, uint32_t *vals_in, uint32_t *vals_out, uint32_t *recpos,
                                    uint2 *post, uint64_t *d_u) {
    rank_new_genes<KeyT>(c, res, off, kmer_off, n, m, n_res, keys_in, vals_in);
    pdl_sort_pairs<KeyT>(c, keys_in, keys_out, vals_in, vals_out, m, c->rp.rank_bits, false, nullptr, 0, c->rp.key_bits == c->rp.rank_bits);
    scan_and_apply(c, m, RecHead<KeyT>{keys_out, vals_out}, RecScatter<KeyT>{keys_out, vals_out, m, recpos, post}, d_u);
    return keys_out;
}
const void *pdl_query_dictionary(pdl_ctx *c, const uint8_t *res, const uint64_t *off, const uint64_t *kmer_off, uint32_t n, uint64_t m,
                                 uint64_t n_res, void *keys_a, void *keys_b, uint32_t *vals_a, uint32_t *vals_b, uint32_t *recpos, uint2 *post,
                                 uint64_t *d_u) {
    if (c->key64) return query_dictionary<uint64_t>(c, res, off, kmer_off, n, m, n_res, (uint64_t *) keys_a, (uint64_t *) keys_b, vals_a, vals_b, recpos, post, d_u);
    return query_dictionary<uint32_t>(c, res, off, kmer_off, n, m, n_res, (uint32_t *) keys_a, (uint32_t *) keys_b, vals_a, vals_b, recpos, post, d_u);
}

template <class KeyT>
static void append_sorted_stream(pdl_ctx *c, uint32_t n, uint64_t m, uint64_t n_res, uint32_t n_base, uint64_t m_base) {
    auto &q = c->qb;
    KeyT *k_in = q.keys_a.as<KeyT>(), *k_out = q.keys_b.as<KeyT>();
    uint32_t *v_in = q.vals_a.as<uint32_t>(), *v_out = q.vals_b.as<uint32_t>();
    ev_begin(c, EV_RANK);
    rank_new_genes<KeyT>(c, q.res.as<uint8_t>(), q.off.as<uint64_t>(), q.koff.as<uint64_t>(), n, m, n_res, k_in, v_in);
    ev_end(c, EV_RANK);
    ev_begin(c, EV_SORT1);
    pdl_sort_pairs<KeyT>(c, k_in, k_out, v_in, v_out, m, c->rp.rank_bits, false, nullptr, 0, c->rp.key_bits == c->rp.rank_bits);
    ev_end(c, EV_SORT1);
    const uint32_t sorted_bits = c->rp.key_bits == c->rp.rank_bits ? 64u : std::min<uint32_t>(64u, 8u * ((c->rp.rank_bits + 7) / 8));
    const KeyT mask = sorted_bits >= 8 * sizeof(KeyT) ? (KeyT) ~(KeyT) 0 : (KeyT) (((KeyT) 1 << (sorted_bits & (8 * sizeof(KeyT) - 1))) - 1);
    ev_begin(c, EV_MERGE);
    pdl_merge_streams<KeyT>(c->stream, c->keys_b.as<KeyT>(), c->vals_b.as<uint32_t>(), (uint32_t) m_base, k_out, v_out, (uint32_t) m, n_base, mask,
                            c->scan_tmp.as<uint32_t>(), c->keys_a.as<KeyT>(), c->vals_a.as<uint32_t>());
    ev_end(c, EV_MERGE);
    c->keys_a.swap(c->keys_b); c->vals_a.swap(c->vals_b);
}

void pdl_run_append(pdl_ctx *c, const uint8_t *residues, const uint64_t *offsets, const uint32_t *genome_ids, uint32_t n, uint32_t n_new_genomes,
                    pdl_append_info *info) {
    hipStream_t st = c->stream;
    auto &q = c->qb;
    const uint32_t N0 = c->N, G0 = c->G;
    const uint64_t M0 = c->M, U0 = c->U;
    if ((uint64_t) N0 + n >= 0x7fffffffull) PDL_FAIL(PDL_ERR_UNSUPPORTED, "%llu genes in the union exceed the 31-bit gene ids", (unsigned long long) N0 + n);
    const uint64_t Rq = offsets[n] - offsets[0];
    if (c->R + Rq >= 0xfffffff0ull) PDL_FAIL(PDL_ERR_UNSUPPORTED, "more than 2^32 residues in the union need 64-bit stream positions");
    const NewGenes genes(offsets, n, c->rp.k);
    const uint64_t m = genes.M;
    if (M0 + m >= 0xfffff000ull) PDL_FAIL(PDL_ERR_UNSUPPORTED, "%llu k-mers in the union need 64-bit stream positions", (unsigned long long) (M0 + m));
    EventSpans<2> &spans = c->app_spans;
    spans.start(st);

    spans.begin();
    q.ctl.alloc(16 * sizeof(uint64_t));
    unsigned long long *d_bad = q.ctl.as<unsigned long long>();
    PDL_HIP(hipMemsetAsync(d_bad, 0, sizeof(uint64_t), st));
    genes.upload(c, residues);
    pdl_check_alphabet(c, q.res.as<uint8_t>(), Rq, d_bad);
    spans.end();
    {
        PinRead rd(c);
        const uint64_t *pb = rd.add<uint64_t>(d_bad, 1);
        rd.sync();
        if (pb[0]) pdl_fail_absent_byte(pb[0], "appended");
    }

    context_changes(c);
    const uint32_t N1 = N0 + n, G1 = G0 + n_new_genomes;
    const uint64_t M1 = M0 + m;
    const size_t kb = c->key64 ? 8 : 4;
    c->kseq_len.grow_keep((size_t) N1 * sizeof(uint32_t), st);
    c->gene_len.grow_keep((size_t) N1 * sizeof(uint32_t), st);
    const bool ids_on_device = c->d_gen && (c->d_gen == c->in_gen.p || c->d_gen == c->ing_gen.p);
    const bool ids_owned = c->d_gen && c->d_gen == c->own_gen.p;
    if (ids_owned) c->own_gen.grow_keep((size_t) N1 * sizeof(uint32_t), st); else c->own_gen.alloc((size_t) N1 * sizeof(uint32_t));
    const uint32_t *old_gen = c->d_gen;
    pdl_extend_layout(c, genome_ids, n);
    c->M = M1; c->R += Rq;
    c->d_gen = c->own_gen.as<uint32_t>(); c->d_res = nullptr; c->d_off = nullptr;
    if (m) {
        c->keys_a.alloc(M1 * kb); c->vals_a.alloc(M1 * sizeof(uint32_t));
        q.keys_a.alloc(m * kb); q.keys_b.alloc(m * kb); q.vals_a.alloc(m * 4); q.vals_b.alloc(m * 4);
        c->scan_tmp.alloc(pdl_merge_split_words(M1) * sizeof(uint32_t));
    }
    c->ev[EV_RANK].used = c->ev[EV_SORT1].used = c->ev[EV_MERGE].used = false;
    rebuild_behind_sort(c, spans, M1, N1, G1, [&] {
        PDL_HIP(hipMemcpyAsync(c->kseq_len.as<uint32_t>() + N0, q.kseq.p, n * 4ull, hipMemcpyDeviceToDevice, st));
        PDL_HIP(hipMemcpyAsync(c->gene_len.as<uint32_t>() + N0, genes.len.data(), n * 4ull, hipMemcpyHostToDevice, st));
        if (ids_owned) {
            PDL_HIP(hipMemcpyAsync(c->own_gen.as<uint32_t>() + N0, c->h_genome_of.data() + N0, n * 4ull, hipMemcpyHostToDevice, st));
        } else if (ids_on_device) {
            PDL_HIP(hipMemcpyAsync(c->own_gen.p, old_gen, (size_t) N0 * 4, hipMemcpyDeviceToDevice, st));
            PDL_HIP(hipMemcpyAsync(c->own_gen.as<uint32_t>() + N0, c->h_genome_of.data() + N0, n * 4ull, hipMemcpyHostToDevice, st));
        } else {
            PDL_HIP(hipMemcpyAsync(c->own_gen.p, c->h_genome_of.data(), (size_t) N1 * 4, hipMemcpyHostToDevice, st));
        }
        if (m) {
            if (c->key64) append_sorted_stream<uint64_t>(c, n, m, Rq, N0, M0);
            else append_sorted_stream<uint32_t>(c, n, m, Rq, N0, M0);
        }
    });
    const float ms0 = spans.ms(0), ms1 = spans.ms(1);
    const float rank_ms = ev_ms(c, EV_RANK), sort_ms = ev_ms(c, EV_SORT1), merge_ms = ev_ms(c, EV_MERGE);
    pdl_timings t{};
// ... 428 lines not shown
```

pandelos_amd/csrc/pdl_groups.h:

```cpp
#pragma once
#include "pdl_common.h"
#include "pdl_scan.h"
#include "pdl_sort.h"

constexpr uint32_t HEAD_BIT = 0x80000000u;
constexpr uint32_t GT_NONE = 0xffffffffu;
constexpr uint32_t COST_LDS_GENOMES = 4096;
constexpr int GW_ROUNDS = 16, GW_TILE = GW_ROUNDS * PDL_WAVE, GW_THREADS = 256, GW_WAVES = GW_THREADS / PDL_WAVE;
constexpr uint32_t GW_MAX_IV = 2048;

__device__ __forceinline__ uint32_t find_head_back(const uint2 *post, uint32_t pos, uint32_t lane) {
    for (;;) {
        const uint32_t base = pos + 1 >= PDL_WAVE ? pos + 1 - PDL_WAVE : 0;
        const uint32_t idx = base + lane;
        const bool f = idx <= pos && ((post[idx <= pos ? idx : pos].y >> 31) || idx == 0);
        const unsigned long long m = __ballot(f);
        if (m) return base + 63u - (uint32_t) __clzll((long long) m);
        pos = base - 1;
    }
}
__device__ __forceinline__ uint32_t find_head_fwd(const uint2 *post, uint32_t pos, uint32_t n, uint32_t lane) {
    for (uint32_t base = pos; base < n; base += PDL_WAVE) {
        const uint32_t idx = base + lane;
        const bool f = idx < n && (post[idx < n ? idx : n - 1].y >> 31);
// ... 266 lines not shown
            gt_round_extent(m[j], t0 + j * PDL_WAVE, lane, nextr[j], pr, gs, ge);
            const bool shared = u < n && ge - gs >= 2;
            n_rec += shared; n_grp += shared && u == gs;
            if constexpr (RECORD_COSTS) { if (shared) atomicAdd(&a.cost[po[j].x], (unsigned long long) (ge - gs)); }
            if constexpr (GENOMES) {
                if (shared) {
                    const uint32_t gen = a.genome_of[po[j].x];
                    const unsigned long long full = ge - gs, up = ge - u - 1;
                    if (lds_table) { atomicAdd(&s_full[gen], full); if (up) atomicAdd(&s_upper[gen], up); }
                    else { atomicAdd(&a.g_full[gen], full); if (up) atomicAdd(&a.g_upper[gen], up); }
                }
            }
        }
    }
    gt_flush_counts<false>(a, s_red, n_rec, n_grp, 0u);
    if constexpr (GENOMES) {
        if (lds_table) for (uint32_t i = tid; i < a.n_genomes; i += GW_THREADS) {
            if (s_full[i]) atomicAdd(&a.g_full[i], s_full[i]);
            if (s_upper[i]) atomicAdd(&a.g_upper[i], s_upper[i]);
        }
    }
}

__global__ __launch_bounds__(256) void k_gene_costs_lazy(const uint2 *__restrict__ post, const unsigned long long *__restrict__ head_bits,
                                                         uint32_t n, unsigned long long *__restrict__ cost) {
    const uint32_t u = blockIdx.x * 256 + threadIdx.x;
    if (u >= n) return;
    const uint32_t w = u >> 6, b = u & 63u, words = (n + 63) >> 6;
    uint32_t gs, ge;
    {
        unsigned long long m = head_bits[w] & ((2ull << b) - 1ull);
        uint32_t ww = w;
        while (!m && ww > 0) m = head_bits[--ww];
        gs = m ? ww * 64u + 63u - (uint32_t) __clzll((long long) m) : 0u;
    }
    {
        unsigned long long m = b == 63 ? 0ull : head_bits[w] & ~((2ull << b) - 1ull);
        uint32_t ww = w;
        while (!m && ww + 1 < words) m = head_bits[++ww];
        ge = m ? ww * 64u + (uint32_t) __ffsll((long long) m) - 1u : n;
        if (ge > n) ge = n;
    }
    if (ge - gs >= 2) atomicAdd(&cost[post[u].x], (unsigned long long) (ge - gs));
}
__global__ __launch_bounds__(256) void k_restore_heads(uint2 *__restrict__ post, const unsigned long long *__restrict__ head_bits, uint32_t n) {
    const uint32_t u = blockIdx.x * 256 + threadIdx.x;
    if (u >= n) return;
    if ((head_bits[u >> 6] >> (u & 63u)) & 1ull) post[u].y |= HEAD_BIT;
}

template <int MODE>
__global__ __launch_bounds__(GW_THREADS) void k_range_count(GroupTileArgs a) {
    extern __shared__ unsigned long long s_dyn[];
    __shared__ uint32_t s_red[2];
    uint2 *s_iv = reinterpret_cast<uint2 *>(s_dyn);
    const uint32_t n_iv = (MODE == 0 || MODE == 2) ? a.n_own_iv : 0u;
    if constexpr (MODE == 0 || MODE == 2) { for (uint32_t i = threadIdx.x; i < n_iv; i += GW_THREADS) s_iv[i] = a.own_iv[i]; }
    if (threadIdx.x < 2) s_red[threadIdx.x] = 0;
    pdl_sync();
    const uint32_t tid = threadIdx.x, lane = tid & (PDL_WAVE - 1);
    const uint32_t gw = blockIdx.x * GW_WAVES + tid / PDL_WAVE;
    const uint32_t n = (uint32_t) scan_count(a.n_bound, a.d_n);
    const uint32_t tiles = (n + GW_TILE - 1) / GW_TILE;
    uint32_t n_rec = 0, n_grp = 0, n_rep = 0;
    for (uint32_t tile = gw; tile < tiles; tile += gridDim.x * GW_WAVES)
        gt_count_tile<MODE, false>(a, tile, n, lane, s_iv, n_iv, nullptr, n_rec, n_grp, n_rep);
    gt_flush_counts<true>(a, s_red, n_rec, n_grp, n_rep);
}

static_assert(GW_WAVES * GW_TILE == (int) PDL_RADIX_TILE && GW_THREADS == (int) PDL_RADIX_BINS, "a workgroup's four tiles are one tile of the radix pass");
__global__ __launch_bounds__(GW_THREADS) void k_range_count_hist(GroupTileArgs a, uint32_t n_tiles4, uint32_t *__restrict__ counts) {
    __shared__ uint32_t s_h[PDL_RADIX_BINS];
    __shared__ uint32_t s_red[2];
    const uint32_t tid = threadIdx.x, lane = tid & (PDL_WAVE - 1), wave = tid / PDL_WAVE;
    const uint32_t n = (uint32_t) scan_count(a.n_bound, a.d_n);
    if (tid < 2) s_red[tid] = 0;
    uint32_t n_rec = 0, n_grp = 0, n_rep = 0;
    for (uint32_t blk = blockIdx.x; blk < n_tiles4; blk += gridDim.x) {
        s_h[tid] = 0;
        pdl_sync();
        const uint32_t tile = blk * GW_WAVES + wave;
        if (tile * GW_TILE < n) gt_count_tile<1, true>(a, tile, n, lane, nullptr, 0u, s_h, n_rec, n_grp, n_rep);
        pdl_sync();
        counts[(size_t) tid * n_tiles4 + blk] = s_h[tid];
    }
    gt_flush_counts<true>(a, s_red, n_rec, n_grp, n_rep);
}

template <int MODE>
__global__ __launch_bounds__(GW_THREADS) void k_group_write(GroupTileArgs a) {
    extern __shared__ unsigned long long s_dyn[];
    __shared__ unsigned long long s_own;
    uint2 *s_iv = reinterpret_cast<uint2 *>(s_dyn);
    const uint32_t n_iv = (MODE == 0 || MODE == 2) ? a.n_own_iv : 0u;
    if constexpr (MODE == 0 || MODE == 2) { for (uint32_t i = threadIdx.x; i < n_iv; i += GW_THREADS) s_iv[i] = a.own_iv[i]; }
    const uint32_t tid = threadIdx.x, lane = tid & (PDL_WAVE - 1);
    const uint32_t gw = blockIdx.x * GW_WAVES + tid / PDL_WAVE;
    const uint32_t n = (uint32_t) scan_count(a.n_bound, a.d_n);
    const uint32_t tiles = (n + GW_TILE - 1) / GW_TILE;
    if (tid == 0) s_own = 0;
    pdl_sync();
    const unsigned long long lt_mask = (1ull << lane) - 1ull;
    unsigned long long own_lookups = 0;
    for (uint32_t tile = gw; tile < tiles; tile += gridDim.x * GW_WAVES) {
        const uint32_t t0 = tile * GW_TILE;
        uint2 po[GW_ROUNDS];
        gt_load_tile(a.post, t0, n, lane, po);
        uint32_t hb, ha;
        gt_load_borders(a, tile, tiles, lane, hb, ha);
        const uint32_t ins = gt_shard_mask<MODE>(a, s_iv, n_iv, po);
        unsigned long long m[GW_ROUNDS];
        gt_head_masks(po, t0, n, lane, m);
        uint32_t before, after;
        gt_tile_borders(a, tile, tiles, t0, n, m[0], lane, hb, ha, before, after);
        uint32_t nextr[GW_ROUNDS];
        gt_next_heads(m, t0, after, nextr);
        uint32_t pr = before, cnt_tile = 0;
        const uint32_t tile_prefix = a.chunk_sums[tile / PDL_WAVE] + a.tile_sums[tile];
#pragma unroll
        for (int j = 0; j < GW_ROUNDS; j++) {
            const uint32_t u = t0 + j * PDL_WAVE + lane;
            uint32_t gs, ge;
            gt_round_extent(m[j], t0 + j * PDL_WAVE, lane, nextr[j], pr, gs, ge);
            const bool live = u < n;
            const bool shared = live && ge - gs >= 2;
            const bool mine = MODE == 1 || ((ins >> j) & 1u);
            bool r = shared && mine;
            if constexpr (MODE == 1 || MODE == 2) r = r && u + 1 < ge;
            const unsigned long long rb = __ballot(r);
            const uint32_t cnt = gt_take_head(a, tile, j, u, live, po[j].y, m[j], lane);
            if (live) {
                if (shared && mine) own_lookups += ge - gs;
                if (r) {
                    const uint32_t at = tile_prefix + cnt_tile + (uint32_t) __popcll(rb & lt_mask);
                    const uint32_t start = MODE == 0 ? gs : u + 1;
                    a.key2[at] = po[j].x;
                    if (a.pay8) a.pay8[at] = gt_pack_range(start, ge - start, cnt, a.pos_base);
                    else a.tuples[at] = make_uint4(start, ge - start, cnt, ge - gs);
                } else if (MODE == 1 || MODE == 2) {
                    if (!a.pay8 && ge - gs >= 2 && u + 1 == ge && mine) atomicAdd(&a.cost[po[j].x], (unsigned long long) (ge - gs));
                }
            }
            cnt_tile += (uint32_t) __popcll(rb);
        }
    }
#pragma unroll
    for (int d = PDL_WAVE / 2; d > 0; d >>= 1) own_lookups += __shfl_xor(own_lookups, d, PDL_WAVE);
    if (lane == 0 && own_lookups) atomicAdd(&s_own, own_lookups);
    pdl_sync();
    if (tid == 0 && s_own) atomicAdd(&a.counters[2], s_own);
}

__global__ __launch_bounds__(GW_THREADS) void k_range_scatter(GroupTileArgs a, uint32_t n_tiles4, const uint32_t *__restrict__ offs,
                                                              uint32_t *__restrict__ keys_out, unsigned long long *__restrict__ vals_out) {
    const uint32_t n = (uint32_t) scan_count(a.n_bound, a.d_n);
    if ((uint64_t) blockIdx.x * PDL_RADIX_TILE >= n) return;
    __shared__ uint32_t s_key[PDL_RADIX_TILE];
    __shared__ unsigned long long s_val[PDL_RADIX_TILE];
    __shared__ uint16_t s_cnt[GW_WAVES][PDL_RADIX_BINS];
    __shared__ uint32_t s_tile_off[PDL_RADIX_BINS];
    __shared__ uint32_t s_goff[PDL_RADIX_BINS];
    __shared__ uint32_t s_wsum[17];
    __shared__ unsigned long long s_own;
    const uint32_t tid = threadIdx.x, lane = tid & (PDL_WAVE - 1), wave = tid / PDL_WAVE;
    const uint32_t tiles = (n + GW_TILE - 1) / GW_TILE;
    const uint32_t tile = blockIdx.x * GW_WAVES + wave, t0 = tile * GW_TILE;
    const bool active = tile < tiles;
    for (int w = 0; w < GW_WAVES; w++) s_cnt[w][tid] = 0;
    s_goff[tid] = offs[(size_t) tid * n_tiles4 + blockIdx.x];
    if (tid == 0) s_own = 0;
    pdl_sync();

    const unsigned long long lt_mask = (1ull << lane) - 1ull;
    uint2 po[GW_ROUNDS];
    unsigned long long val[GW_ROUNDS];
    uint16_t rank[GW_ROUNDS];
    uint32_t rbits = 0;
    unsigned long long own_lookups = 0;
    gt_load_tile(a.post, t0, n, lane, po);
    if (active) {
        uint32_t hb, ha;
        gt_load_borders(a, tile, tiles, lane, hb, ha);
        unsigned long long m[GW_ROUNDS];
        gt_head_masks(po, t0, n, lane, m);
        uint32_t before, after;
        gt_tile_borders(a, tile, tiles, t0, n, m[0], lane, hb, ha, before, after);
        uint32_t nextr[GW_ROUNDS];
        gt_next_heads(m, t0, after, nextr);
        uint32_t pr = before;
#pragma unroll
        for (int j = 0; j < GW_ROUNDS; j++) {
            const uint32_t u = t0 + j * PDL_WAVE + lane;
            uint32_t gs, ge;
            gt_round_extent(m[j], t0 + j * PDL_WAVE, lane, nextr[j], pr, gs, ge);
            const bool live = u < n;
            const bool shared = live && ge - gs >= 2;
            const bool r = shared && u + 1 < ge;
            const uint32_t cnt = gt_take_head(a, tile, j, u, live, po[j].y, m[j], lane);
            if (shared) own_lookups += ge - gs;
            val[j] = gt_pack_range(u + 1, ge - u - 1, cnt, 0u);
            rbits |= (uint32_t) r << j;
        }
    }
#pragma unroll
    for (int j = 0; j < GW_ROUNDS; j++) {
        const bool valid = (rbits >> j) & 1u;
        const uint32_t d = po[j].x & (PDL_RADIX_BINS - 1);
        unsigned long long same = __ballot(valid);
#pragma unroll
        for (int b = 0; b < 8; b++) {
            const unsigned long long mb = __ballot((d >> b) & 1u);
            same &= ((d >> b) & 1u) ? mb : ~mb;
        }
        const uint32_t seen = s_cnt[wave][d];
        rank[j] = (uint16_t) (seen + (uint32_t) __popcll(same & lt_mask));
        if (valid && (same & lt_mask) == 0) s_cnt[wave][d] = (uint16_t) (seen + (uint32_t) __popcll(same));
    }
    pdl_sync();
    uint32_t tot = 0;
    uint32_t wcnt[GW_WAVES];
#pragma unroll
    for (int w = 0; w < GW_WAVES; w++) { wcnt[w] = s_cnt[w][tid]; tot += wcnt[w]; }
    uint32_t tile_total;
    const uint32_t ex = block_exclusive_scan_u32(tot, s_wsum, tile_total);
    s_tile_off[tid] = ex;
    uint32_t run = ex;
#pragma unroll
    for (int w = 0; w < GW_WAVES; w++) { s_cnt[w][tid] = (uint16_t) run; run += wcnt[w]; }
    pdl_sync();
#pragma unroll
    for (int j = 0; j < GW_ROUNDS; j++) {
        if ((rbits >> j) & 1u) {
            const uint32_t lp = s_cnt[wave][po[j].x & (PDL_RADIX_BINS - 1)] + rank[j];
            s_key[lp] = po[j].x;
            s_val[lp] = val[j];
        }
    }
#pragma unroll
    for (int d = PDL_WAVE / 2; d > 0; d >>= 1) own_lookups += __shfl_xor(own_lookups, d, PDL_WAVE);
    if (lane == 0 && own_lookups) atomicAdd(&s_own, own_lookups);
    pdl_sync();
#pragma unroll
    for (int j = 0; j < GW_ROUNDS; j++) {
        const uint32_t e = j * GW_THREADS + tid;
        if (e < tile_total) {
            const uint32_t k = s_key[e];
            const uint32_t d = k & (PDL_RADIX_BINS - 1);
            const uint64_t dst = (uint64_t) s_goff[d] + (e - s_tile_off[d]);
            keys_out[dst] = k;
            vals_out[dst] = s_val[e];
        }
    }
    if (tid == 0 && s_own) atomicAdd(&a.counters[2], s_own);
}

__global__ __launch_bounds__(256) void k_tile_prefix(uint32_t *__restrict__ tile_sums, const uint64_t *d_n, uint64_t n_bound,
                                                     uint32_t *__restrict__ chunk_sums, uint32_t n_blocks) {
    const uint32_t b = blockIdx.x * 4 + threadIdx.x / PDL_WAVE, lane = threadIdx.x & (PDL_WAVE - 1);
    if (b >= n_blocks) return;
    const uint32_t tiles = (uint32_t) ((scan_count(n_bound, d_n) + GW_TILE - 1) / GW_TILE);
    const uint32_t t = b * PDL_WAVE + lane;
    const uint32_t v = t < tiles ? tile_sums[t] : 0u;
    const uint32_t inc = wave_inclusive_scan_u32(v);
    if (t < tiles) tile_sums[t] = inc - v;
    if (lane == PDL_WAVE - 1) chunk_sums[b] = inc;
}

static uint32_t group_tiles_plan(pdl_ctx *c, GroupTileArgs &a) {
    const uint64_t tiles = (a.n_bound + GW_TILE - 1) / GW_TILE;
    if (tiles > 0x7fffffffull) PDL_FAIL(PDL_ERR_UNSUPPORTED, "dictionary of %llu records exceeds the grid limit", (unsigned long long) a.n_bound);
    const int cus = pdl_cus(c);
    a.n_blocks = (uint32_t) ((tiles + PDL_WAVE - 1) / PDL_WAVE);
    const uint32_t grid = (uint32_t) std::max<uint64_t>(1, std::min<uint64_t>((tiles + GW_WAVES - 1) / GW_WAVES, (uint64_t) cus * 8));
    c->scan_tmp.alloc(((size_t) tiles * 3 + a.n_blocks + 1) * sizeof(uint32_t));
    a.tile_sums = c->scan_tmp.as<uint32_t>(); a.th_first = a.tile_sums + tiles; a.th_last = a.th_first + tiles; a.chunk_sums = a.th_last + tiles;
    return grid;
}
template <bool GENOMES, bool RECORD_COSTS>
static void launch_group_costs(pdl_ctx *c, const GroupTileArgs &a, uint32_t grid) {
    const size_t dyn = GENOMES && a.n_genomes <= COST_LDS_GENOMES ? 2 * (size_t) a.n_genomes * sizeof(uint64_t) : 0;
    hipLaunchKernelGGL((k_group_costs<GENOMES, RECORD_COSTS>), dim3(grid), dim3(GW_THREADS), dyn, c->stream, a);
    PDL_HIP(hipGetLastError());
}
template <class F>
static void with_range_mode(int mode, F &&f) {
    if (mode == 1) f(std::integral_constant<int, 1>{});
    else if (mode == 2) f(std::integral_constant<int, 2>{});
    else f(std::integral_constant<int, 0>{});
}
static void launch_range_count(pdl_ctx *c, const GroupTileArgs &a, uint32_t grid, int mode) {
    const size_t dyn = (size_t) a.n_own_iv * sizeof(uint2);
    with_range_mode(mode, [&](auto m) { hipLaunchKernelGGL(k_range_count<decltype(m)::value>, dim3(grid), dim3(GW_THREADS), dyn, c->stream, a); });
    hipLaunchKernelGGL(k_tile_prefix, dim3((a.n_blocks + 3) / 4), dim3(256), 0, c->stream, a.tile_sums, a.d_n, a.n_bound, a.chunk_sums, a.n_blocks);
    hipLaunchKernelGGL(k_scan_tile_scan, dim3(1), dim3(1024), 0, c->stream, a.chunk_sums, a.n_blocks, c->scalars.as<uint64_t>() + PDL_CTL_RANGES, (uint64_t *) nullptr);
    PDL_HIP(hipGetLastError());
}
static void launch_range_write(pdl_ctx *c, const GroupTileArgs &a, uint32_t grid, int mode) {
    const size_t dyn = (size_t) a.n_own_iv * sizeof(uint2);
    with_range_mode(mode, [&](auto m) { hipLaunchKernelGGL(k_group_write<decltype(m)::value>, dim3(grid), dim3(GW_THREADS), dyn, c->stream, a); });
    PDL_HIP(hipGetLastError());
}
```

pandelos_amd/csrc/pdl_scan.h:

```cpp
#pragma once

#include "pdl_common.h"

#include <type_traits>

template <class T, class = void> struct scan_two_phase : std::false_type {};
template <class T> struct scan_two_phase<T, std::void_t<typename T::Loaded>> : std::true_type {};

constexpr int SCAN_THREADS = 256;
constexpr int SCAN_ITEMS = 8;
constexpr int SCAN_TILE = SCAN_THREADS * SCAN_ITEMS;

__device__ __forceinline__ uint32_t wave_inclusive_scan_u32(uint32_t v) {
    const int lane = threadIdx.x & (PDL_WAVE - 1);
#pragma unroll
    for (int d = 1; d < PDL_WAVE; d <<= 1) {
        uint32_t o = __shfl_up(v, d, PDL_WAVE);
        if (lane >= d) v += o;
    }
    return v;
}

__device__ __forceinline__ uint32_t block_exclusive_scan_u32(uint32_t v, uint32_t *s_wave , uint32_t &total) {
    const int lane = threadIdx.x & (PDL_WAVE - 1);
    const int wave = threadIdx.x / PDL_WAVE;
    const int nw = blockDim.x / PDL_WAVE;
    uint32_t inc = wave_inclusive_scan_u32(v);
    if (lane == PDL_WAVE - 1) s_wave[wave] = inc;
    pdl_sync();
    if (threadIdx.x == 0) {
        uint32_t run = 0;
        for (int w = 0; w < nw; w++) { uint32_t t = s_wave[w]; s_wave[w] = run; run += t; }
        s_wave[16] = run;
    }
    pdl_sync();
    uint32_t res = inc - v + s_wave[wave];
    total = s_wave[16];
    pdl_sync();
    return res;
}

__device__ __forceinline__ uint64_t scan_count(uint64_t n, const uint64_t *d_n) {
    if (!d_n) return n;
    const uint64_t v = *d_n;
    return v < n ? v : n;
}

template <class FlagF>
__global__ __launch_bounds__(SCAN_THREADS) void k_scan_tile_sums(FlagF flag, uint64_t n_bound, const uint64_t *d_n, uint32_t *tile_sums) {
    __shared__ uint32_t s_wave[17];
    const uint64_t n = scan_count(n_bound, d_n);
    if ((uint64_t) blockIdx.x * SCAN_TILE >= n) {
        if (threadIdx.x == 0) tile_sums[blockIdx.x] = 0;
        return;
    }
    const uint64_t base = (uint64_t) blockIdx.x * SCAN_TILE;
    uint32_t sum = 0;
#pragma unroll
    for (int j = 0; j < SCAN_ITEMS; j++) {
        const uint64_t i = base + (uint64_t) j * SCAN_THREADS + threadIdx.x;
        const uint32_t f = flag(i < n ? i : n - 1);
        sum += i < n ? f : 0u;
    }
    uint32_t total;
    (void) block_exclusive_scan_u32(sum, s_wave, total);
    if (threadIdx.x == 0) tile_sums[blockIdx.x] = total;
}

static __global__ __launch_bounds__(1024) void k_scan_tile_scan(uint32_t *tile_sums, uint32_t n_tiles, uint64_t *d_total, uint64_t *d_total2) {
    __shared__ uint32_t s_wave[17];
    __shared__ uint32_t s_carry;
    if (threadIdx.x == 0) s_carry = 0;
    pdl_sync();
    for (uint32_t base = 0; base < n_tiles; base += 1024) {
        uint32_t i = base + threadIdx.x;
        uint32_t v = i < n_tiles ? tile_sums[i] : 0;
        uint32_t total;
        uint32_t ex = block_exclusive_scan_u32(v, s_wave, total);
        uint32_t carry = s_carry;
        if (i < n_tiles) tile_sums[i] = ex + carry;
        pdl_sync();
        if (threadIdx.x == 0) s_carry = carry + total;
        pdl_sync();
    }
    if (threadIdx.x == 0) {
        *d_total = s_carry;
        if (d_total2) {
            reinterpret_cast<uint32_t *>(d_total2)[0] = s_carry;
            reinterpret_cast<uint32_t *>(d_total2)[1] = 0u;
        }
    }
}

constexpr uint32_t SCAN_INLINE_TILES = 1024;
template <class FlagF, class ApplyF, bool INLINE_PREFIX>
__global__ __launch_bounds__(SCAN_THREADS) void k_scan_apply(FlagF flag, ApplyF apply, uint64_t n_bound, const uint64_t *d_n, const uint32_t *tile_sums,
                                                            uint64_t *d_total, uint64_t *d_total2) {
    __shared__ uint32_t s_flags[SCAN_TILE];
    __shared__ uint32_t s_pref[SCAN_TILE];
    __shared__ uint32_t s_wave[17];
    const uint64_t n = scan_count(n_bound, d_n);
    const uint64_t base = (uint64_t) blockIdx.x * SCAN_TILE;
    uint32_t tile_prefix = 0;
    if constexpr (INLINE_PREFIX) {
        const uint32_t upto = blockIdx.x == 0 ? gridDim.x : blockIdx.x;
        uint32_t part = 0;
        for (uint32_t i = threadIdx.x; i < upto; i += SCAN_THREADS) part += tile_sums[i];
        uint32_t all;
        (void) block_exclusive_scan_u32(part, s_wave, all);
        if (blockIdx.x == 0) {
            if (threadIdx.x == 0) {
                *d_total = all;
                if (d_total2) { reinterpret_cast<uint32_t *>(d_total2)[0] = all; reinterpret_cast<uint32_t *>(d_total2)[1] = 0u; }
            }
        } else {
            tile_prefix = all;
        }
    } else {
        tile_prefix = tile_sums[blockIdx.x];
    }
    if (base >= n) return;
#pragma unroll
    for (int j = 0; j < SCAN_ITEMS; j++) {
        const uint32_t li = j * SCAN_THREADS + threadIdx.x;
        const uint64_t i = base + li;
        const uint32_t f = flag(i < n ? i : n - 1);
        s_flags[li] = i < n ? f : 0u;
    }
    pdl_sync();
    uint32_t f[SCAN_ITEMS];
    uint32_t sum = 0;
#pragma unroll
    for (int j = 0; j < SCAN_ITEMS; j++) { f[j] = s_flags[threadIdx.x * SCAN_ITEMS + j]; sum += f[j]; }
    uint32_t total;
    uint32_t prefix = block_exclusive_scan_u32(sum, s_wave, total) + tile_prefix;
#pragma unroll
    for (int j = 0; j < SCAN_ITEMS; j++) { s_pref[threadIdx.x * SCAN_ITEMS + j] = prefix; prefix += f[j]; }
    pdl_sync();
    if constexpr (scan_two_phase<ApplyF>::value) {
        typename ApplyF::Loaded v[SCAN_ITEMS];
#pragma unroll
        for (int j = 0; j < SCAN_ITEMS; j++) {
            const uint32_t li = j * SCAN_THREADS + threadIdx.x;
            const uint64_t i = base + li;
            v[j] = apply.load(i < n ? i : n - 1, s_flags[li]);
        }
#pragma unroll
        for (int j = 0; j < SCAN_ITEMS; j++) {
            const uint32_t li = j * SCAN_THREADS + threadIdx.x;
            const uint64_t i = base + li;
            if (i < n) apply.store(i, s_flags[li], s_pref[li], v[j]);
        }
    } else {
#pragma unroll
        for (int j = 0; j < SCAN_ITEMS; j++) {
            uint32_t li = j * SCAN_THREADS + threadIdx.x;
            uint64_t i = base + li;
            if (i < n) apply(i, s_flags[li], s_pref[li]);
        }
    }
}

constexpr uint32_t LB_CHUNK = PDL_WAVE;
constexpr uint32_t LB_MAX_POLLS = 1u << 22;
constexpr uint32_t LB_CTR_WORDS = 16;
struct LookbackArgs {
    unsigned long long *tile_agg, *chunk_agg, *chunk_incl;
    uint32_t *ctr;
    uint32_t epoch;
};
__device__ __forceinline__ unsigned long long lb_pack(uint32_t epoch, uint32_t value) { return (unsigned long long) epoch << 32 | value; }
__device__ __forceinline__ void lb_publish(unsigned long long *p, uint32_t epoch, uint32_t value) {
    __hip_atomic_store(p, lb_pack(epoch, value), __ATOMIC_RELAXED, __HIP_MEMORY_SCOPE_AGENT);
}
__device__ __forceinline__ uint32_t lb_wait(const unsigned long long *p, uint32_t epoch, uint32_t *err) {
    for (uint32_t polls = 0;; polls++) {
        const unsigned long long w = __hip_atomic_load(p, __ATOMIC_RELAXED, __HIP_MEMORY_SCOPE_AGENT);
        if ((uint32_t) (w >> 32) == epoch) return (uint32_t) w;
        if (polls >= LB_MAX_POLLS) { atomicAdd(err, 1u); return 0u; }
        __builtin_amdgcn_s_sleep(1);
    }
}
__device__ __forceinline__ uint32_t lb_wave_sum(uint32_t v) {
#pragma unroll
    for (int d = PDL_WAVE / 2; d > 0; d >>= 1) v += __shfl_xor(v, d, PDL_WAVE);
    return v;
}
__device__ __forceinline__ uint32_t lb_tile_prefix(const LookbackArgs &lb, uint32_t tile, uint32_t tiles, uint32_t total) {
    const uint32_t lane = threadIdx.x & (PDL_WAVE - 1);
    const uint32_t c = tile / LB_CHUNK, i = tile % LB_CHUNK;
    uint32_t *err = lb.ctr + 2;
    if (lane == 0) lb_publish(&lb.tile_agg[tile], lb.epoch, total);
    const uint32_t in_chunk = min(LB_CHUNK, tiles - c * LB_CHUNK);
    const bool completes = i == in_chunk - 1;
    const uint32_t v = lane < i ? lb_wait(&lb.tile_agg[c * LB_CHUNK + lane], lb.epoch, err) : 0u;
    const uint32_t within = lb_wave_sum(v);
    const uint32_t chunk_sum = within + total;
    if (completes && lane == 0) lb_publish(&lb.chunk_agg[c], lb.epoch, chunk_sum);
    uint32_t before = 0;
    for (uint32_t base = c; base > 0;) {
        const bool live = lane < base;
        const uint32_t cc = live ? base - 1 - lane : 0u;
        const unsigned long long wi = live ? __hip_atomic_load(&lb.chunk_incl[cc], __ATOMIC_RELAXED, __HIP_MEMORY_SCOPE_AGENT) : 0ull;
        const bool has_incl = live && (uint32_t) (wi >> 32) == lb.epoch;
        const unsigned long long mi = __ballot(has_incl);
        const uint32_t first = mi ? (uint32_t) __ffsll((long long) mi) - 1u : PDL_WAVE;
        uint32_t part = 0;
        if (live && lane < first) part = lb_wait(&lb.chunk_agg[cc], lb.epoch, err);
        if (lane == first) part = (uint32_t) wi;
        before += lb_wave_sum(part);
        if (mi || base <= PDL_WAVE) break;
        base -= PDL_WAVE;
    }
    if (lane == 0) {
        if (i == 0 && c > 0) lb_publish(&lb.chunk_incl[c - 1], lb.epoch, before);
        if (completes) lb_publish(&lb.chunk_incl[c], lb.epoch, before + chunk_sum);
    }
    return before + within;
}
template <class FlagF, class ApplyF>
__global__ __launch_bounds__(SCAN_THREADS) void k_scan_onepass(FlagF flag, ApplyF apply, uint64_t n_bound, const uint64_t *d_n, LookbackArgs lb,
                                                               uint32_t n_chunks_bound, uint64_t *d_total, uint64_t *d_total2) {
    __shared__ uint32_t s_flags[SCAN_TILE];
    __shared__ uint32_t s_pref[SCAN_TILE];
    __shared__ uint32_t s_wave[17];
    __shared__ uint32_t s_prefix;
    const uint64_t n = scan_count(n_bound, d_n);
    const uint32_t tiles = (uint32_t) ((n + SCAN_TILE - 1) / SCAN_TILE);
    const uint32_t tile = blockIdx.x;
    if (tile < tiles) {
        const uint64_t base = (uint64_t) tile * SCAN_TILE;
#pragma unroll
        for (int j = 0; j < SCAN_ITEMS; j++) {
            const uint32_t li = j * SCAN_THREADS + threadIdx.x;
            const uint64_t i = base + li;
            const uint32_t f = flag(i < n ? i : n - 1);
            s_flags[li] = i < n ? f : 0u;
        }
        pdl_sync();
        uint32_t f[SCAN_ITEMS];
        uint32_t sum = 0;
#pragma unroll
        for (int j = 0; j < SCAN_ITEMS; j++) { f[j] = s_flags[threadIdx.x * SCAN_ITEMS + j]; sum += f[j]; }
        uint32_t total;
// ... 104 lines not shown
```

pandelos_amd/csrc/pdl_sort.h:

```cpp
#pragma once

#include "pdl_common.h"

template <class KeyT, class ValT = uint32_t>
void pdl_sort_pairs(pdl_ctx *c, KeyT *&keys_in, KeyT *&keys_out, ValT *&vals_in, ValT *&vals_out,
                    uint64_t n, uint32_t end_bit, bool iota_values = false,
                    const uint64_t *d_n = nullptr,
                    uint32_t begin_bit = 0,
                    bool keys_below_end_bit = false);

constexpr uint32_t PDL_RADIX_TILE = 4096, PDL_RADIX_BINS = 256;
void pdl_radix_offsets(pdl_ctx *c, const uint32_t *counts, uint32_t *offs, uint32_t n_tiles, uint64_t *d_total);

extern template void pdl_sort_pairs<uint32_t, uint32_t>(pdl_ctx *, uint32_t *&, uint32_t *&, uint32_t *&, uint32_t *&, uint64_t, uint32_t, bool, const uint64_t *, uint32_t, bool);
extern template void pdl_sort_pairs<uint64_t, uint32_t>(pdl_ctx *, uint64_t *&, uint64_t *&, uint32_t *&, uint32_t *&, uint64_t, uint32_t, bool, const uint64_t *, uint32_t, bool);
extern template void pdl_sort_pairs<uint32_t, unsigned long long>(pdl_ctx *, uint32_t *&, uint32_t *&, unsigned long long *&, unsigned long long *&, uint64_t, uint32_t, bool, const uint64_t *, uint32_t, bool);
```

pandelos_amd/csrc/pdl_sort.hip:

```cpp
#include "pdl_sort.h"
#include "pdl_scan.h"

constexpr int RS_THREADS = 256;
constexpr int RS_WAVES = RS_THREADS / PDL_WAVE;
constexpr int RS_ROUNDS = 16;
constexpr int RS_TILE = RS_THREADS * RS_ROUNDS;
constexpr int RS_WAVE_SPAN = PDL_WAVE * RS_ROUNDS;
constexpr int RS_BINS = 256;
static_assert(RS_THREADS == RS_BINS, "one thread per digit in the tile-level scans");

template <class KeyT>
__device__ __forceinline__ uint32_t rs_digit(KeyT k, uint32_t shift) { return (uint32_t) (k >> shift) & 0xffu; }

template <class KeyT>
__global__ __launch_bounds__(RS_THREADS) void k_rs_hist(const KeyT *__restrict__ keys, uint64_t n_bound, const uint64_t *d_n, uint32_t shift,
                                                        uint32_t n_tiles, uint32_t *__restrict__ counts) {
    __shared__ uint32_t s_h[RS_BINS];
    const uint64_t n = scan_count(n_bound, d_n);
    const uint64_t base = (uint64_t) blockIdx.x * RS_TILE;
    if (base >= n) {
        counts[(size_t) threadIdx.x * n_tiles + blockIdx.x] = 0;
        return;
    }
    s_h[threadIdx.x] = 0;
    pdl_sync();
    KeyT key[RS_ROUNDS];
#pragma unroll
    for (int j = 0; j < RS_ROUNDS; j++) {
        const uint64_t i = base + (uint64_t) j * RS_THREADS + threadIdx.x;
        key[j] = keys[i < n ? i : n - 1];
    }
#pragma unroll
    for (int j = 0; j < RS_ROUNDS; j++) {
        const uint64_t i = base + (uint64_t) j * RS_THREADS + threadIdx.x;
        if (i < n) atomicAdd(&s_h[rs_digit(key[j], shift)], 1u);
    }
    pdl_sync();
    counts[(size_t) threadIdx.x * n_tiles + blockIdx.x] = s_h[threadIdx.x];
}

struct RsCountFlag {
    const uint32_t *counts;
    __device__ uint32_t operator()(uint64_t i) const { return counts[i]; }
};
struct RsOffsApply {
    uint32_t *offs;
    __device__ void operator()(uint64_t i, uint32_t, uint32_t prefix) const { offs[i] = prefix; }
};

template <class KeyT, class ValT>
__global__ __launch_bounds__(RS_THREADS) void k_rs_scatter(const KeyT *__restrict__ keys_in, const ValT *vals_in,
                                                           KeyT *__restrict__ keys_out, ValT *__restrict__ vals_out, uint64_t n_bound,
                                                           const uint64_t *d_n, uint32_t shift, uint32_t n_tiles, const uint32_t *__restrict__ offs,
                                                           uint32_t nbits) {
    const uint64_t n = scan_count(n_bound, d_n);
    if ((uint64_t) blockIdx.x * (RS_THREADS * RS_ROUNDS) >= n) return;
    __shared__ KeyT s_key[RS_TILE];
    __shared__ ValT s_val[RS_TILE];
    __shared__ uint32_t s_cnt[RS_WAVES][RS_BINS];
    __shared__ uint32_t s_tile_off[RS_BINS];
    __shared__ uint32_t s_goff[RS_BINS];
    __shared__ uint32_t s_wsum[17];

    const uint32_t tid = threadIdx.x, lane = tid & (PDL_WAVE - 1), wave = tid / PDL_WAVE;
    const uint64_t tile_base = (uint64_t) blockIdx.x * RS_TILE;
    const uint64_t wave_base = tile_base + (uint64_t) wave * RS_WAVE_SPAN;
    for (int w = 0; w < RS_WAVES; w++) s_cnt[w][tid] = 0;
    s_goff[tid] = offs[(size_t) tid * n_tiles + blockIdx.x];
    pdl_sync();

    KeyT key[RS_ROUNDS];
    ValT val[RS_ROUNDS];
    uint16_t rank[RS_ROUNDS];
#pragma unroll
    for (int j = 0; j < RS_ROUNDS; j++) {
        const uint64_t i = wave_base + (uint64_t) j * PDL_WAVE + lane;
        key[j] = keys_in[i < n ? i : n - 1];
    }
    if (vals_in) {
#pragma unroll
        for (int j = 0; j < RS_ROUNDS; j++) {
            const uint64_t i = wave_base + (uint64_t) j * PDL_WAVE + lane;
            val[j] = vals_in[i < n ? i : n - 1];
        }
    } else {
#pragma unroll
        for (int j = 0; j < RS_ROUNDS; j++) val[j] = (ValT) (wave_base + (uint64_t) j * PDL_WAVE + lane);
    }
#pragma unroll
    for (int j = 0; j < RS_ROUNDS; j++) {
        const uint64_t i = wave_base + (uint64_t) j * PDL_WAVE + lane;
        const bool valid = i < n;
        const uint32_t d = rs_digit(key[j], shift);
        unsigned long long same = __ballot(valid);
#pragma unroll
        for (int b = 0; b < 8; b++) {
            if ((uint32_t) b >= nbits) break;
            const unsigned long long m = __ballot((d >> b) & 1u);
            same &= ((d >> b) & 1u) ? m : ~m;
        }
        const uint32_t before = s_cnt[wave][d];
        const uint32_t below_me = __builtin_amdgcn_mbcnt_hi((uint32_t) (same >> 32), __builtin_amdgcn_mbcnt_lo((uint32_t) same, 0u));
        rank[j] = (uint16_t) (before + below_me);
        if (valid && below_me == 0) s_cnt[wave][d] = before + (uint32_t) __popcll(same);
    }
    pdl_sync();
    uint32_t tot = 0;
    uint32_t wcnt[RS_WAVES];
#pragma unroll
    for (int w = 0; w < RS_WAVES; w++) { wcnt[w] = s_cnt[w][tid]; tot += wcnt[w]; }
    uint32_t tile_total;
    const uint32_t ex = block_exclusive_scan_u32(tot, s_wsum, tile_total);
    s_tile_off[tid] = ex;
    uint32_t run = ex;
#pragma unroll
    for (int w = 0; w < RS_WAVES; w++) { s_cnt[w][tid] = run; run += wcnt[w]; }
    pdl_sync();
#pragma unroll
    for (int j = 0; j < RS_ROUNDS; j++) {
        const uint64_t i = wave_base + (uint64_t) j * PDL_WAVE + lane;
        if (i < n) {
            const uint32_t lp = s_cnt[wave][rs_digit(key[j], shift)] + rank[j];
            s_key[lp] = key[j];
            s_val[lp] = val[j];
        }
    }
    pdl_sync();
#pragma unroll
    for (int j = 0; j < RS_ROUNDS; j++) {
        const uint32_t e = j * RS_THREADS + tid;
        if (e < tile_total) {
            const KeyT k = s_key[e];
            const uint32_t d = rs_digit(k, shift);
            const uint64_t dst = (uint64_t) s_goff[d] + (e - s_tile_off[d]);
            keys_out[dst] = k;
            vals_out[dst] = s_val[e];
        }
    }
}

template <class KeyT, class ValT>
void pdl_sort_pairs(pdl_ctx *c, KeyT *&keys_in, KeyT *&keys_out, ValT *&vals_in, ValT *&vals_out,
                    uint64_t n, uint32_t end_bit, bool iota_values, const uint64_t *d_n, uint32_t begin_bit, bool keys_below_end_bit) {
    if (n == 0) return;
    if (end_bit == 0) end_bit = 1;
    if (end_bit > sizeof(KeyT) * 8) end_bit = sizeof(KeyT) * 8;
    if (n >= 0xfffff000ull) PDL_FAIL(PDL_ERR_UNSUPPORTED, "sort of %llu pairs needs 64-bit positions", (unsigned long long) n);
    const uint32_t n_tiles = (uint32_t) ((n + RS_TILE - 1) / RS_TILE);
    const size_t table = (size_t) RS_BINS * n_tiles;
    c->sort_tmp.alloc(2 * table * sizeof(uint32_t));
    uint32_t *counts = c->sort_tmp.as<uint32_t>(), *offs = counts + table;
    uint64_t *d_total = c->scalars.as<uint64_t>() + PDL_CTL_SCAN_TOTAL;
    const uint32_t passes = (end_bit + 7) / 8;
    for (uint32_t p = begin_bit / 8; p < passes; p++) {
        const uint32_t shift = p * 8;
        hipLaunchKernelGGL((k_rs_hist<KeyT>), dim3(n_tiles), dim3(RS_THREADS), 0, c->stream, keys_in, n, d_n, shift, n_tiles, counts);
        scan_and_apply(c, table, RsCountFlag{counts}, RsOffsApply{offs}, d_total);
        hipLaunchKernelGGL((k_rs_scatter<KeyT, ValT>), dim3(n_tiles), dim3(RS_THREADS), 0, c->stream, keys_in,
                           (p == begin_bit / 8 && iota_values) ? (const ValT *) nullptr : vals_in, keys_out, vals_out, n, d_n, shift, n_tiles, offs,
                           keys_below_end_bit ? std::min<uint32_t>(8, end_bit - shift) : 8u);
        PDL_HIP(hipGetLastError());
        std::swap(keys_in, keys_out);
        std::swap(vals_in, vals_out);
    }
    std::swap(keys_in, keys_out);
    std::swap(vals_in, vals_out);
}

void pdl_radix_offsets(pdl_ctx *c, const uint32_t *counts, uint32_t *offs, uint32_t n_tiles, uint64_t *d_total) {
    static_assert(PDL_RADIX_TILE == RS_TILE && PDL_RADIX_BINS == RS_BINS, "the caller's kernels use the tile shape of the sort");
    scan_and_apply(c, (size_t) RS_BINS * n_tiles, RsCountFlag{counts}, RsOffsApply{offs}, d_total);
}

template void pdl_sort_pairs<uint32_t, uint32_t>(pdl_ctx *, uint32_t *&, uint32_t *&, uint32_t *&, uint32_t *&, uint64_t, uint32_t, bool, const uint64_t *, uint32_t, bool);
template void pdl_sort_pairs<uint64_t, uint32_t>(pdl_ctx *, uint64_t *&, uint64_t *&, uint32_t *&, uint32_t *&, uint64_t, uint32_t, bool, const uint64_t *, uint32_t, bool);
template void pdl_sort_pairs<uint32_t, unsigned long long>(pdl_ctx *, uint32_t *&, uint32_t *&, unsigned long long *&, unsigned long long *&, uint64_t, uint32_t, bool, const uint64_t *, uint32_t, bool);
```

Before: 1438 billion.

## Add lean radix path: per-digit offset scan, fused rank histogram, wave-parallel searches

Adds a lean radix-sort mode, on by default. The multi-kernel global scan over the counts table is replaced with one kernel that scans each digit's row independently and records per-digit totals, and the scatter kernels fold the cross-digit base into their in-tile scan by packing tile and digit counts into 64-bit words. The rank kernel gains a mode that computes the first sort pass's histogram while emitting keys, so that pass's separate histogram kernel is skipped. Boundary binary searches and small-span sequence lookups now use wave-wide ballots, and the tile-sum scan gets a single-pass fast path. These changes target launch count and memory traffic in dictionary sorting; the 13-bit packing and the tile limit constrain which sizes qualify.

```diff
diff --git a/pandelos_amd/csrc/pdl_api.hip b/pandelos_amd/csrc/pdl_api.hip
--- a/pandelos_amd/csrc/pdl_api.hip
+++ b/pandelos_amd/csrc/pdl_api.hip
@@ -750,6 +750,7 @@
     else if (n == "staging_cap") c->opt_staging_cap = value > 0 ? (uint64_t) value : 0;
     else if (n == "aside_test_reload") c->opt_aside_test_reload = value != 0;
     else if (n == "onepass_scan") c->opt_onepass_scan = value != 0;
+    else if (n == "lean_radix") c->opt_lean_radix = value != 0;
     else if (n == "low_memory") c->opt_low_memory = value != 0;
     else if (n == "query_batch_bytes") {
         if (value <= 0) { c->err = "query_batch_bytes: a positive byte count"; return PDL_ERR_ARGUMENT; }
diff --git a/pandelos_amd/csrc/pdl_common.h b/pandelos_amd/csrc/pdl_common.h
--- a/pandelos_amd/csrc/pdl_common.h
+++ b/pandelos_amd/csrc/pdl_common.h
@@ -287,6 +287,7 @@
     bool opt_low_memory = false;
     bool reshard_pending = false;
     bool opt_onepass_scan = false;
+    bool opt_lean_radix = true;
     DevBuf scratch;
     DevBuf scalars;
 
diff --git a/pandelos_amd/csrc/pdl_dict.hip b/pandelos_amd/csrc/pdl_dict.hip
--- a/pandelos_amd/csrc/pdl_dict.hip
+++ b/pandelos_amd/csrc/pdl_dict.hip
@@ -122,24 +122,49 @@
 
 constexpr uint32_t DIST_BIN_BITS = 12, DIST_BINS = 1u << DIST_BIN_BITS;
 
+__device__ __forceinline__ uint32_t wave_upper_bound_u64(const uint64_t *a, uint32_t lo, uint32_t hi, uint64_t v) {
+    const uint32_t lane = threadIdx.x & (PDL_WAVE - 1);
+    while (hi - lo > PDL_WAVE) {
+        const uint32_t step = (hi - lo + PDL_WAVE - 1) / PDL_WAVE;
+        const uint64_t at = (uint64_t) lo + (uint64_t) lane * step;
+        const bool le = at < hi && a[at] <= v;
+        const uint32_t c = (uint32_t) __popcll(__ballot(le));
+        if (c == 0) return lo;
+        const uint64_t next = (uint64_t) lo + (uint64_t) c * step;
+        if (next < hi) hi = (uint32_t) next;
+        lo = lo + (c - 1) * step + 1;
+    }
+    const bool le = lo + lane < hi && a[lo + lane] <= v;
+    return lo + (uint32_t) __popcll(__ballot(le));
+}
+
 template <class KeyT, int MODE>
 __global__ __launch_bounds__(RANK_THREADS) void k_rank(const uint8_t *__restrict__ res, const uint64_t *__restrict__ off,
                                                        const uint64_t *__restrict__ kmer_off, uint32_t n_seq, uint64_t m, uint64_t n_res,
                                                        RankParams rp, KeyT *__restrict__ keys, uint32_t *__restrict__ vals,
                                                        uint32_t bin_shift, uint32_t *__restrict__ bins) {
+    static_assert(RANK_THREADS == (int) PDL_RADIX_BINS && PDL_RADIX_TILE % RANK_TILE == 0, "MODE 2: one thread per byte value, whole trips per radix tile");
+    constexpr uint32_t TRIPS = MODE == 2 ? PDL_RADIX_TILE / RANK_TILE : 1;
+    constexpr uint64_t TILE = (uint64_t) RANK_TILE * TRIPS;
     __shared__ uint8_t s_rv[256];
     __shared__ uint32_t s_lo, s_hi;
     __shared__ uint64_t s_koff[RANK_SPAN + 1], s_off[RANK_SPAN];
-    __shared__ uint32_t s_bins[MODE == 1 ? DIST_BINS : 1];
+    __shared__ uint32_t s_bins[MODE == 1 ? DIST_BINS : MODE == 2 ? PDL_RADIX_BINS : 1];
     for (int i = threadIdx.x; i < 256; i += RANK_THREADS) s_rv[i] = rp.rank_values[i];
     if constexpr (MODE == 1) for (uint32_t i = threadIdx.x; i < DIST_BINS; i += RANK_THREADS) s_bins[i] = 0;
-    const uint64_t tiles = (m + RANK_TILE - 1) / RANK_TILE;
+    const uint64_t tiles = (m + TILE - 1) / TILE;
   for (uint64_t tile = blockIdx.x; tile < tiles; tile += gridDim.x) {
     pdl_sync();
-    const uint64_t q0 = tile * RANK_TILE;
-    const uint64_t q_last = min(q0 + RANK_TILE, m) - 1;
-    if (threadIdx.x == 0) s_lo = upper_bound_u64(kmer_off, 0, n_seq + 1, q0) - 1;
-    if (threadIdx.x == 64) s_hi = upper_bound_u64(kmer_off, 0, n_seq + 1, q_last) - 1;
+    const uint64_t q0 = tile * TILE;
+    const uint64_t q_last = min(q0 + TILE, m) - 1;
+    if (threadIdx.x < PDL_WAVE) {
+        const uint32_t b = wave_upper_bound_u64(kmer_off, 0, n_seq + 1, q0) - 1;
+        if (threadIdx.x == 0) s_lo = b;
+    } else if (threadIdx.x < 2 * PDL_WAVE) {
+        const uint32_t b = wave_upper_bound_u64(kmer_off, 0, n_seq + 1, q_last) - 1;
+        if (threadIdx.x == PDL_WAVE) s_hi = b;
+    }
+    if constexpr (MODE == 2) s_bins[threadIdx.x] = 0;
     pdl_sync();
     const uint32_t lo = s_lo, hi = s_hi;
     const uint32_t span = hi - lo + 1;
@@ -149,19 +174,26 @@
         for (uint32_t i = threadIdx.x; i < span; i += RANK_THREADS) s_off[i] = off[lo + i];
     }
     pdl_sync();
+    const uint64_t my_koff = staged ? s_koff[min(threadIdx.x & (PDL_WAVE - 1), span)] : 0;
+#pragma unroll 1
+   for (uint32_t trip = 0; trip < TRIPS; trip++) {
+    const uint64_t qt0 = q0 + (uint64_t) trip * RANK_TILE;
+    if (qt0 >= m) break;
     const uint32_t k = rp.k;
     const KeyT base = (KeyT) rp.base;
     uint32_t sq[RANK_ITEMS];
     uint64_t pos[RANK_ITEMS];
 #pragma unroll
     for (int j = 0; j < RANK_ITEMS; j++) {
-        const uint64_t qj = q0 + (uint64_t) j * RANK_THREADS + threadIdx.x;
+        const uint64_t qj = qt0 + (uint64_t) j * RANK_THREADS + threadIdx.x;
         const uint64_t q = qj < m ? qj : m - 1;
         if (staged) {
             uint32_t a = 0;
-            if (span <= 8) {
-#pragma unroll
-                for (uint32_t i = 1; i < 8; i++) a += (uint32_t) (i < span && s_koff[i < span ? i : 0] <= q);
+            if (span <= PDL_WAVE) {
+                const uint64_t qf = min(qt0 + (uint64_t) j * RANK_THREADS + (threadIdx.x & ~(PDL_WAVE - 1)), m - 1), ql = min(qf + PDL_WAVE - 1, m - 1);
+                const uint32_t a0 = (uint32_t) __popcll(__ballot(my_koff <= qf)) - 1, a1 = (uint32_t) __popcll(__ballot(my_koff <= ql)) - 1;
+                a = a0;
+                for (uint32_t i = a0 + 1; i <= a1; i++) a += (uint32_t) (s_koff[i] <= q);
             } else {
                 uint32_t b = span;
                 while (a < b) { const uint32_t mid = (a + b) >> 1; if (s_koff[mid + 1] <= q) a = mid + 1; else b = mid; }
@@ -196,11 +228,17 @@
     }
 #pragma unroll
     for (int j = 0; j < RANK_ITEMS; j++) {
-        const uint64_t q = q0 + (uint64_t) j * RANK_THREADS + threadIdx.x;
+        const uint64_t q = qt0 + (uint64_t) j * RANK_THREADS + threadIdx.x;
         if (q < m) {
             if constexpr (MODE == 1) atomicAdd(&s_bins[(uint32_t) (r[j] >> bin_shift)], 1u);
+            if constexpr (MODE == 2) atomicAdd(&s_bins[(uint32_t) r[j] & (PDL_RADIX_BINS - 1)], 1u);
             keys[q] = r[j]; vals[q] = sq[j];
         }
+    }
+   }
+    if constexpr (MODE == 2) {
+        pdl_sync();
+        bins[(size_t) threadIdx.x * tiles + tile] = s_bins[threadIdx.x];
     }
   }
     if constexpr (MODE == 1) {
@@ -442,7 +480,7 @@
 }
 
 template <class KeyT>
-static void stage_rank(pdl_ctx *c, uint32_t *d_bins = nullptr, uint32_t bin_shift = 0) {
+static bool stage_rank(pdl_ctx *c, uint32_t *d_bins = nullptr, uint32_t bin_shift = 0) {
     hipStream_t st = c->stream;
     const uint64_t M = c->M;
     c->keys_a.alloc(M * sizeof(KeyT)); c->keys_b.alloc(M * sizeof(KeyT));
@@ -458,10 +496,18 @@
         const uint64_t tiles = (M + RANK_TILE - 1) / RANK_TILE;
         if (d_bins) hipLaunchKernelGGL((k_rank<KeyT, 1>), dim3((uint32_t) std::min<uint64_t>(tiles, 2048)), dim3(RANK_THREADS), 0, st, c->d_res, c->d_off,
                                        c->kmer_off.as<uint64_t>(), c->N, M, c->R, c->rp, c->keys_a.as<KeyT>(), c->vals_a.as<uint32_t>(), bin_shift, d_bins);
+        else if (pdl_radix_lean(c, M)) {
+            c->sort_tmp.alloc(pdl_radix_tmp_bytes(M));
+            hipLaunchKernelGGL((k_rank<KeyT, 2>), dim3((uint32_t) ((M + PDL_RADIX_TILE - 1) / PDL_RADIX_TILE)), dim3(RANK_THREADS), 0, st, c->d_res, c->d_off,
+                               c->kmer_off.as<uint64_t>(), c->N, M, c->R, c->rp, c->keys_a.as<KeyT>(), c->vals_a.as<uint32_t>(), 0u, c->sort_tmp.as<uint32_t>());
+            PDL_HIP(hipGetLastError());
+            return true;
+        }
         else hipLaunchKernelGGL((k_rank<KeyT, 0>), dim3((uint32_t) tiles), dim3(RANK_THREADS), 0, st, c->d_res, c->d_off,
                                 c->kmer_off.as<uint64_t>(), c->N, M, c->R, c->rp, c->keys_a.as<KeyT>(), c->vals_a.as<uint32_t>(), 0u, (uint32_t *) nullptr);
     }
     PDL_HIP(hipGetLastError());
+    return false;
 }
 
 template <class KeyT>
@@ -477,9 +523,10 @@
 }
 
 template <class KeyT>
-static void stage_sort_and_dedup(pdl_ctx *c, KeyT *keys_in, KeyT *keys_out, uint32_t *vals_in, uint32_t *vals_out, uint64_t m) {
+static void stage_sort_and_dedup(pdl_ctx *c, KeyT *keys_in, KeyT *keys_out, uint32_t *vals_in, uint32_t *vals_out, uint64_t m,
+                                 bool first_counts_filed = false) {
     ev_begin(c, EV_SORT1);
-    pdl_sort_pairs<KeyT>(c, keys_in, keys_out, vals_in, vals_out, m, c->rp.rank_bits, false, nullptr, 0, c->rp.key_bits == c->rp.rank_bits);
+    pdl_sort_pairs<KeyT>(c, keys_in, keys_out, vals_in, vals_out, m, c->rp.rank_bits, false, nullptr, 0, c->rp.key_bits == c->rp.rank_bits, first_counts_filed);
     ev_end(c, EV_SORT1);
     if ((void *) keys_out != c->keys_b.p) c->keys_a.swap(c->keys_b);
     if ((void *) vals_out != c->vals_b.p) c->vals_a.swap(c->vals_b);
@@ -559,13 +606,13 @@
         if (fused) {
             const uint32_t n_tiles4 = (uint32_t) ((bound + PDL_RADIX_TILE - 1) / PDL_RADIX_TILE);
             const size_t table = (size_t) PDL_RADIX_BINS * n_tiles4, tiles = (bound + GW_TILE - 1) / GW_TILE;
-            c->sort_tmp.alloc((2 * table + 3 * tiles + 1) * sizeof(uint32_t));
-            uint32_t *counts = c->sort_tmp.as<uint32_t>(), *offs = counts + table;
-            ga.tile_sums = offs + table; ga.th_first = ga.tile_sums + tiles; ga.th_last = ga.th_first + tiles; ga.chunk_sums = nullptr;
+            c->sort_tmp.alloc((2 * table + PDL_RADIX_BINS + 3 * tiles + 1) * sizeof(uint32_t));
+            uint32_t *counts = c->sort_tmp.as<uint32_t>(), *offs = counts + table, *digit_total = offs + table;
+            ga.tile_sums = digit_total + PDL_RADIX_BINS; ga.th_first = ga.tile_sums + tiles; ga.th_last = ga.th_first + tiles; ga.chunk_sums = nullptr;
             const uint32_t grid4 = std::max<uint32_t>(1, std::min<uint32_t>(n_tiles4, (uint32_t) c->cus * 8));
             hipLaunchKernelGGL(k_range_count_hist, dim3(grid4), dim3(GW_THREADS), 0, st, ga, n_tiles4, counts);
-            pdl_radix_offsets(c, counts, offs, n_tiles4, d_scal + PDL_CTL_RANGES);
-            hipLaunchKernelGGL(k_range_scatter, dim3(n_tiles4), dim3(GW_THREADS), 0, st, ga, n_tiles4, offs, k2b, pay_b);
+            const uint32_t *totals = pdl_radix_offsets(c, counts, offs, n_tiles4, d_scal + PDL_CTL_RANGES, digit_total);
+            hipLaunchKernelGGL(k_range_scatter, dim3(n_tiles4), dim3(GW_THREADS), 0, st, ga, n_tiles4, offs, k2b, pay_b, totals, d_scal + PDL_CTL_RANGES);
             PDL_HIP(hipGetLastError());
         } else {
         launch_range_count(c, ga, grid, mode);
@@ -686,11 +733,11 @@
 static void dictionary_pipeline(pdl_ctx *c, bool only_complexity) {
     const uint64_t M = c->M;
     ev_begin(c, EV_RANK);
-    stage_rank<KeyT>(c);
+    const bool counts_filed = stage_rank<KeyT>(c);
     ev_end(c, EV_RANK);
     KeyT *keys_in = c->keys_a.as<KeyT>(), *keys_out = c->keys_b.as<KeyT>();
     uint32_t *vals_in = c->vals_a.as<uint32_t>(), *vals_out = c->vals_b.as<uint32_t>();
-    stage_sort_and_dedup<KeyT>(c, keys_in, keys_out, vals_in, vals_out, M);
+    stage_sort_and_dedup<KeyT>(c, keys_in, keys_out, vals_in, vals_out, M, counts_filed);
     ev_end(c, EV_DICT);
     if (c->layout_deferred) pdl_finish_layout(c);
     if (!only_complexity) pdl_prepare_tasks(c);
diff --git a/pandelos_amd/csrc/pdl_groups.h b/pandelos_amd/csrc/pdl_groups.h
--- a/pandelos_amd/csrc/pdl_groups.h
+++ b/pandelos_amd/csrc/pdl_groups.h
@@ -442,22 +442,27 @@
 }
 
 __global__ __launch_bounds__(GW_THREADS) void k_range_scatter(GroupTileArgs a, uint32_t n_tiles4, const uint32_t *__restrict__ offs,
-                                                              uint32_t *__restrict__ keys_out, unsigned long long *__restrict__ vals_out) {
+                                                              uint32_t *__restrict__ keys_out, unsigned long long *__restrict__ vals_out,
+                                                              const uint32_t *__restrict__ digit_total, uint64_t *d_total) {
     const uint32_t n = (uint32_t) scan_count(a.n_bound, a.d_n);
-    if ((uint64_t) blockIdx.x * PDL_RADIX_TILE >= n) return;
+    if ((uint64_t) blockIdx.x * PDL_RADIX_TILE >= n) {
+        if (digit_total && blockIdx.x == 0 && threadIdx.x == 0) *d_total = 0;
+        return;
+    }
     __shared__ uint32_t s_key[PDL_RADIX_TILE];
     __shared__ unsigned long long s_val[PDL_RADIX_TILE];
     __shared__ uint16_t s_cnt[GW_WAVES][PDL_RADIX_BINS];
     __shared__ uint32_t s_tile_off[PDL_RADIX_BINS];
     __shared__ uint32_t s_goff[PDL_RADIX_BINS];
-    __shared__ uint32_t s_wsum[17];
+    __shared__ unsigned long long s_wsum[17];
     __shared__ unsigned long long s_own;
     const uint32_t tid = threadIdx.x, lane = tid & (PDL_WAVE - 1), wave = tid / PDL_WAVE;
     const uint32_t tiles = (n + GW_TILE - 1) / GW_TILE;
     const uint32_t tile = blockIdx.x * GW_WAVES + wave, t0 = tile * GW_TILE;
     const bool active = tile < tiles;
     for (int w = 0; w < GW_WAVES; w++) s_cnt[w][tid] = 0;
-    s_goff[tid] = offs[(size_t) tid * n_tiles4 + blockIdx.x];
+    const uint32_t goff = offs[(size_t) tid * n_tiles4 + blockIdx.x];
+    const uint32_t dtot = digit_total ? digit_total[tid] : 0u;
     if (tid == 0) s_own = 0;
     pdl_sync();
 
@@ -511,9 +516,11 @@
     uint32_t wcnt[GW_WAVES];
 #pragma unroll
     for (int w = 0; w < GW_WAVES; w++) { wcnt[w] = s_cnt[w][tid]; tot += wcnt[w]; }
-    uint32_t tile_total;
-    const uint32_t ex = block_exclusive_scan_u32(tot, s_wsum, tile_total);
+    uint32_t tile_total, digit_base, grand_total;
+    const uint32_t ex = radix_tile_scan(tot, dtot, s_wsum, tile_total, digit_base, grand_total);
     s_tile_off[tid] = ex;
+    s_goff[tid] = goff + digit_base;
+    if (digit_total && blockIdx.x == 0 && tid == 0) *d_total = grand_total;
     uint32_t run = ex;
 #pragma unroll
     for (int w = 0; w < GW_WAVES; w++) { s_cnt[w][tid] = (uint16_t) run; run += wcnt[w]; }
diff --git a/pandelos_amd/csrc/pdl_scan.h b/pandelos_amd/csrc/pdl_scan.h
--- a/pandelos_amd/csrc/pdl_scan.h
+++ b/pandelos_amd/csrc/pdl_scan.h
@@ -38,6 +38,33 @@
     total = s_wave[16];
     pdl_sync();
     return res;
+}
+
+__device__ __forceinline__ uint32_t radix_tile_scan(uint32_t tile_cnt, uint32_t digit_tot, unsigned long long *s_wave , uint32_t &tile_total,
+                                                    uint32_t &digit_base, uint32_t &grand_total) {
+    const int lane = threadIdx.x & (PDL_WAVE - 1);
+    const int wave = threadIdx.x / PDL_WAVE;
+    const int nw = blockDim.x / PDL_WAVE;
+    const unsigned long long v = (unsigned long long) digit_tot << 13 | tile_cnt;
+    unsigned long long inc = v;
+#pragma unroll
+    for (int d = 1; d < PDL_WAVE; d <<= 1) {
+        const unsigned long long o = __shfl_up(inc, d, PDL_WAVE);
+        if (lane >= d) inc += o;
+    }
+    if (lane == PDL_WAVE - 1) s_wave[wave] = inc;
+    pdl_sync();
+    if (threadIdx.x == 0) {
+        unsigned long long run = 0;
+        for (int w = 0; w < nw; w++) { const unsigned long long t = s_wave[w]; s_wave[w] = run; run += t; }
+        s_wave[16] = run;
+    }
+    pdl_sync();
+    const unsigned long long res = inc - v + s_wave[wave], all = s_wave[16];
+    pdl_sync();
+    tile_total = (uint32_t) all & 0x1fffu; grand_total = (uint32_t) (all >> 13);
+    digit_base = (uint32_t) (res >> 13);
+    return (uint32_t) res & 0x1fffu;
 }
 
 __device__ __forceinline__ uint64_t scan_count(uint64_t n, const uint64_t *d_n) {
@@ -67,9 +94,29 @@
     if (threadIdx.x == 0) tile_sums[blockIdx.x] = total;
 }
 
+constexpr int TS_ITEMS = 16;
+__device__ __forceinline__ void scan_write_totals(uint32_t total, uint64_t *d_total, uint64_t *d_total2) {
+    *d_total = total;
+    if (d_total2) {
+        reinterpret_cast<uint32_t *>(d_total2)[0] = total;
+        reinterpret_cast<uint32_t *>(d_total2)[1] = 0u;
+    }
+}
 static __global__ __launch_bounds__(1024) void k_scan_tile_scan(uint32_t *tile_sums, uint32_t n_tiles, uint64_t *d_total, uint64_t *d_total2) {
     __shared__ uint32_t s_wave[17];
     __shared__ uint32_t s_carry;
+    if (n_tiles <= 1024u * TS_ITEMS) {
+        const uint32_t i0 = threadIdx.x * TS_ITEMS;
+        uint32_t v[TS_ITEMS], sum = 0;
+#pragma unroll
+        for (int j = 0; j < TS_ITEMS; j++) { v[j] = i0 + j < n_tiles ? tile_sums[i0 + j] : 0u; sum += v[j]; }
+        uint32_t total;
+        uint32_t ex = block_exclusive_scan_u32(sum, s_wave, total);
+#pragma unroll
+        for (int j = 0; j < TS_ITEMS; j++) { if (i0 + j < n_tiles) tile_sums[i0 + j] = ex; ex += v[j]; }
+        if (threadIdx.x == 0) scan_write_totals(total, d_total, d_total2);
+        return;
+    }
     if (threadIdx.x == 0) s_carry = 0;
     pdl_sync();
     for (uint32_t base = 0; base < n_tiles; base += 1024) {
@@ -83,13 +130,7 @@
         if (threadIdx.x == 0) s_carry = carry + total;
         pdl_sync();
     }
-    if (threadIdx.x == 0) {
-        *d_total = s_carry;
-        if (d_total2) {
-            reinterpret_cast<uint32_t *>(d_total2)[0] = s_carry;
-            reinterpret_cast<uint32_t *>(d_total2)[1] = 0u;
-        }
-    }
+    if (threadIdx.x == 0) scan_write_totals(s_carry, d_total, d_total2);
 }
 
 constexpr uint32_t SCAN_INLINE_TILES = 1024;
diff --git a/pandelos_amd/csrc/pdl_sort.h b/pandelos_amd/csrc/pdl_sort.h
--- a/pandelos_amd/csrc/pdl_sort.h
+++ b/pandelos_amd/csrc/pdl_sort.h
@@ -7,11 +7,16 @@
                     uint64_t n, uint32_t end_bit, bool iota_values = false,
                     const uint64_t *d_n = nullptr,
                     uint32_t begin_bit = 0,
-                    bool keys_below_end_bit = false);
+                    bool keys_below_end_bit = false,
+                    bool first_counts_filed = false);
 
 constexpr uint32_t PDL_RADIX_TILE = 4096, PDL_RADIX_BINS = 256;
-void pdl_radix_offsets(pdl_ctx *c, const uint32_t *counts, uint32_t *offs, uint32_t n_tiles, uint64_t *d_total);
+const uint32_t *pdl_radix_offsets(pdl_ctx *c, const uint32_t *counts, uint32_t *offs, uint32_t n_tiles, uint64_t *d_total, uint32_t *digit_total);
+bool pdl_radix_lean(const pdl_ctx *c, uint64_t n);
+inline size_t pdl_radix_tmp_bytes(uint64_t n) {
+    return (2 * (size_t) PDL_RADIX_BINS * ((n + PDL_RADIX_TILE - 1) / PDL_RADIX_TILE) + PDL_RADIX_BINS) * sizeof(uint32_t);
+}
 
-extern template void pdl_sort_pairs<uint32_t, uint32_t>(pdl_ctx *, uint32_t *&, uint32_t *&, uint32_t *&, uint32_t *&, uint64_t, uint32_t, bool, const uint64_t *, uint32_t, bool);
-extern template void pdl_sort_pairs<uint64_t, uint32_t>(pdl_ctx *, uint64_t *&, uint64_t *&, uint32_t *&, uint32_t *&, uint64_t, uint32_t, bool, const uint64_t *, uint32_t, bool);
-extern template void pdl_sort_pairs<uint32_t, unsigned long long>(pdl_ctx *, uint32_t *&, uint32_t *&, unsigned long long *&, unsigned long long *&, uint64_t, uint32_t, bool, const uint64_t *, uint32_t, bool);
+extern template void pdl_sort_pairs<uint32_t, uint32_t>(pdl_ctx *, uint32_t *&, uint32_t *&, uint32_t *&, uint32_t *&, uint64_t, uint32_t, bool, const uint64_t *, uint32_t, bool, bool);
+extern template void pdl_sort_pairs<uint64_t, uint32_t>(pdl_ctx *, uint64_t *&, uint64_t *&, uint32_t *&, uint32_t *&, uint64_t, uint32_t, bool, const uint64_t *, uint32_t, bool, bool);
+extern template void pdl_sort_pairs<uint32_t, unsigned long long>(pdl_ctx *, uint32_t *&, uint32_t *&, unsigned long long *&, unsigned long long *&, uint64_t, uint32_t, bool, const uint64_t *, uint32_t, bool, bool);
diff --git a/pandelos_amd/csrc/pdl_sort.hip b/pandelos_amd/csrc/pdl_sort.hip
--- a/pandelos_amd/csrc/pdl_sort.hip
+++ b/pandelos_amd/csrc/pdl_sort.hip
@@ -48,25 +48,52 @@
     __device__ void operator()(uint64_t i, uint32_t, uint32_t prefix) const { offs[i] = prefix; }
 };
 
+constexpr int RO_THREADS = 1024, RO_ITEMS = 4, RO_TRIP = RO_THREADS * RO_ITEMS;
+constexpr uint32_t RO_MAX_TILES = 65536;
+__global__ __launch_bounds__(RO_THREADS) void k_rs_offsets(const uint32_t *__restrict__ counts, uint32_t *__restrict__ offs, uint32_t n_tiles,
+                                                           uint32_t *__restrict__ digit_total) {
+    __shared__ uint32_t s_wave[17];
+    const uint32_t *row = counts + (size_t) blockIdx.x * n_tiles;
+    uint32_t *out = offs + (size_t) blockIdx.x * n_tiles;
+    uint32_t carry = 0;
+    for (uint32_t base = 0; base < n_tiles; base += RO_TRIP) {
+        const uint32_t i0 = base + threadIdx.x * RO_ITEMS;
+        uint32_t v[RO_ITEMS], sum = 0;
+#pragma unroll
+        for (int j = 0; j < RO_ITEMS; j++) { v[j] = i0 + j < n_tiles ? row[i0 + j] : 0u; sum += v[j]; }
+        uint32_t total;
+        uint32_t ex = block_exclusive_scan_u32(sum, s_wave, total) + carry;
+#pragma unroll
+        for (int j = 0; j < RO_ITEMS; j++) { if (i0 + j < n_tiles) out[i0 + j] = ex; ex += v[j]; }
+        carry += total;
+    }
+    if (threadIdx.x == 0) digit_total[blockIdx.x] = carry;
+}
+
 template <class KeyT, class ValT>
 __global__ __launch_bounds__(RS_THREADS) void k_rs_scatter(const KeyT *__restrict__ keys_in, const ValT *vals_in,
                                                            KeyT *__restrict__ keys_out, ValT *__restrict__ vals_out, uint64_t n_bound,
                                                            const uint64_t *d_n, uint32_t shift, uint32_t n_tiles, const uint32_t *__restrict__ offs,
-                                                           uint32_t nbits) {
+                                                           uint32_t nbits,
+                                                           const uint32_t *__restrict__ digit_total, uint64_t *d_total) {
     const uint64_t n = scan_count(n_bound, d_n);
-    if ((uint64_t) blockIdx.x * (RS_THREADS * RS_ROUNDS) >= n) return;
+    if ((uint64_t) blockIdx.x * (RS_THREADS * RS_ROUNDS) >= n) {
+        if (digit_total && blockIdx.x == 0 && threadIdx.x == 0) *d_total = 0;
+        return;
+    }
     __shared__ KeyT s_key[RS_TILE];
     __shared__ ValT s_val[RS_TILE];
     __shared__ uint32_t s_cnt[RS_WAVES][RS_BINS];
     __shared__ uint32_t s_tile_off[RS_BINS];
     __shared__ uint32_t s_goff[RS_BINS];
-    __shared__ uint32_t s_wsum[17];
+    __shared__ unsigned long long s_wsum[17];
 
     const uint32_t tid = threadIdx.x, lane = tid & (PDL_WAVE - 1), wave = tid / PDL_WAVE;
     const uint64_t tile_base = (uint64_t) blockIdx.x * RS_TILE;
     const uint64_t wave_base = tile_base + (uint64_t) wave * RS_WAVE_SPAN;
     for (int w = 0; w < RS_WAVES; w++) s_cnt[w][tid] = 0;
-    s_goff[tid] = offs[(size_t) tid * n_tiles + blockIdx.x];
+    const uint32_t goff = offs[(size_t) tid * n_tiles + blockIdx.x];
+    const uint32_t dtot = digit_total ? digit_total[tid] : 0u;
     pdl_sync();
 
     KeyT key[RS_ROUNDS];
@@ -109,9 +136,11 @@
     uint32_t wcnt[RS_WAVES];
 #pragma unroll
     for (int w = 0; w < RS_WAVES; w++) { wcnt[w] = s_cnt[w][tid]; tot += wcnt[w]; }
-    uint32_t tile_total;
-    const uint32_t ex = block_exclusive_scan_u32(tot, s_wsum, tile_total);
+    uint32_t tile_total, digit_base, grand_total;
+    const uint32_t ex = radix_tile_scan(tot, dtot, s_wsum, tile_total, digit_base, grand_total);
     s_tile_off[tid] = ex;
+    s_goff[tid] = goff + digit_base;
+    if (digit_total && blockIdx.x == 0 && tid == 0) *d_total = grand_total;
     uint32_t run = ex;
 #pragma unroll
     for (int w = 0; w < RS_WAVES; w++) { s_cnt[w][tid] = run; run += wcnt[w]; }
@@ -141,24 +170,26 @@
 
 template <class KeyT, class ValT>
 void pdl_sort_pairs(pdl_ctx *c, KeyT *&keys_in, KeyT *&keys_out, ValT *&vals_in, ValT *&vals_out,
-                    uint64_t n, uint32_t end_bit, bool iota_values, const uint64_t *d_n, uint32_t begin_bit, bool keys_below_end_bit) {
+                    uint64_t n, uint32_t end_bit, bool iota_values, const uint64_t *d_n, uint32_t begin_bit, bool keys_below_end_bit,
+                    bool first_counts_filed) {
     if (n == 0) return;
     if (end_bit == 0) end_bit = 1;
     if (end_bit > sizeof(KeyT) * 8) end_bit = sizeof(KeyT) * 8;
     if (n >= 0xfffff000ull) PDL_FAIL(PDL_ERR_UNSUPPORTED, "sort of %llu pairs needs 64-bit positions", (unsigned long long) n);
     const uint32_t n_tiles = (uint32_t) ((n + RS_TILE - 1) / RS_TILE);
     const size_t table = (size_t) RS_BINS * n_tiles;
-    c->sort_tmp.alloc(2 * table * sizeof(uint32_t));
-    uint32_t *counts = c->sort_tmp.as<uint32_t>(), *offs = counts + table;
+    c->sort_tmp.alloc(pdl_radix_tmp_bytes(n));
+    uint32_t *counts = c->sort_tmp.as<uint32_t>(), *offs = counts + table, *digit_total = offs + table;
     uint64_t *d_total = c->scalars.as<uint64_t>() + PDL_CTL_SCAN_TOTAL;
     const uint32_t passes = (end_bit + 7) / 8;
     for (uint32_t p = begin_bit / 8; p < passes; p++) {
         const uint32_t shift = p * 8;
-        hipLaunchKernelGGL((k_rs_hist<KeyT>), dim3(n_tiles), dim3(RS_THREADS), 0, c->stream, keys_in, n, d_n, shift, n_tiles, counts);
-        scan_and_apply(c, table, RsCountFlag{counts}, RsOffsApply{offs}, d_total);
+        if (!(first_counts_filed && p == begin_bit / 8))
+            hipLaunchKernelGGL((k_rs_hist<KeyT>), dim3(n_tiles), dim3(RS_THREADS), 0, c->stream, keys_in, n, d_n, shift, n_tiles, counts);
+        const uint32_t *totals = pdl_radix_offsets(c, counts, offs, n_tiles, d_total, digit_total);
         hipLaunchKernelGGL((k_rs_scatter<KeyT, ValT>), dim3(n_tiles), dim3(RS_THREADS), 0, c->stream, keys_in,
                            (p == begin_bit / 8 && iota_values) ? (const ValT *) nullptr : vals_in, keys_out, vals_out, n, d_n, shift, n_tiles, offs,
-                           keys_below_end_bit ? std::min<uint32_t>(8, end_bit - shift) : 8u);
+                           keys_below_end_bit ? std::min<uint32_t>(8, end_bit - shift) : 8u, totals, d_total);
         PDL_HIP(hipGetLastError());
         std::swap(keys_in, keys_out);
         std::swap(vals_in, vals_out);
@@ -167,11 +198,21 @@
     std::swap(vals_in, vals_out);
 }
 
-void pdl_radix_offsets(pdl_ctx *c, const uint32_t *counts, uint32_t *offs, uint32_t n_tiles, uint64_t *d_total) {
+bool pdl_radix_lean(const pdl_ctx *c, uint64_t n) {
+    return c->opt_lean_radix && !c->opt_onepass_scan && (n + RS_TILE - 1) / RS_TILE <= RO_MAX_TILES;
+}
+
+const uint32_t *pdl_radix_offsets(pdl_ctx *c, const uint32_t *counts, uint32_t *offs, uint32_t n_tiles, uint64_t *d_total, uint32_t *digit_total) {
     static_assert(PDL_RADIX_TILE == RS_TILE && PDL_RADIX_BINS == RS_BINS, "the caller's kernels use the tile shape of the sort");
-    scan_and_apply(c, (size_t) RS_BINS * n_tiles, RsCountFlag{counts}, RsOffsApply{offs}, d_total);
-}
-
-template void pdl_sort_pairs<uint32_t, uint32_t>(pdl_ctx *, uint32_t *&, uint32_t *&, uint32_t *&, uint32_t *&, uint64_t, uint32_t, bool, const uint64_t *, uint32_t, bool);
-template void pdl_sort_pairs<uint64_t, uint32_t>(pdl_ctx *, uint64_t *&, uint64_t *&, uint32_t *&, uint32_t *&, uint64_t, uint32_t, bool, const uint64_t *, uint32_t, bool);
-template void pdl_sort_pairs<uint32_t, unsigned long long>(pdl_ctx *, uint32_t *&, uint32_t *&, unsigned long long *&, unsigned long long *&, uint64_t, uint32_t, bool, const uint64_t *, uint32_t, bool);
+    if (!pdl_radix_lean(c, (uint64_t) n_tiles * RS_TILE)) {
+        scan_and_apply(c, (size_t) RS_BINS * n_tiles, RsCountFlag{counts}, RsOffsApply{offs}, d_total);
+        return nullptr;
+    }
+    hipLaunchKernelGGL(k_rs_offsets, dim3(RS_BINS), dim3(RO_THREADS), 0, c->stream, counts, offs, n_tiles, digit_total);
+    PDL_HIP(hipGetLastError());
+    return digit_total;
+}
+
+template void pdl_sort_pairs<uint32_t, uint32_t>(pdl_ctx *, uint32_t *&, uint32_t *&, uint32_t *&, uint32_t *&, uint64_t, uint32_t, bool, const uint64_t *, uint32_t, bool, bool);
+template void pdl_sort_pairs<uint64_t, uint32_t>(pdl_ctx *, uint64_t *&, uint64_t *&, uint32_t *&, uint32_t *&, uint64_t, uint32_t, bool, const uint64_t *, uint32_t, bool, bool);
+template void pdl_sort_pairs<uint32_t, unsigned long long>(pdl_ctx *, uint32_t *&, uint32_t *&, unsigned long long *&, unsigned long long *&, uint64_t, uint32_t, bool, const uint64_t *, uint32_t, bool, bool);
```

New measurement: 1476 billion, median of 6. 1.03x the previous value.
